# rueberger/MJHMC

Measured on AMD Instinct MI355X. Metric: particle-steps/sec (ndims x nparticles x L), higher is better.
Workload: dtype f64 state (ProductOfT: around the f32 matrix-core force)

## Files before the change

mjhmc_amd/csrc/api.hip:

```cpp
#include <hip/hip_runtime.h>

#include <algorithm>
#include <atomic>
#include <chrono>
#include <cmath>
#include <cstdio>
#include <cstdlib>
#include <cstring>
#include <string>
#include <thread>
#include <type_traits>
#include <vector>

#include "autocor.hpp"
#include "lagcov.hpp"
#include "handles.hpp"

static thread_local std::string g_err;

int mjhmc_fail(int code, const std::string& msg) {
  g_err = msg;
  return code;
}
static int fail(int code, const std::string& msg) { return mjhmc_fail(code, msg); }
// ... 180 lines not shown
    const int d = d0 + threadIdx.x;
    if (d < D && p < N) dst[(size_t)p * pitch + d] = (T)tile[threadIdx.x][pp];
  }
}

template <typename T>
__global__ void to_dim_major(const T* __restrict__ src, const int64_t* __restrict__ idx, double* __restrict__ dst,
                             int D, int64_t ncols, int pitch, int64_t rs, int64_t cs, int64_t off) {
  __shared__ double tile[32][33];
  const int64_t k0 = (int64_t)blockIdx.x * 32;
  const int d0 = blockIdx.y * 32;
#pragma unroll
  for (int i = 0; i < 4; ++i) {
    const int kk = threadIdx.y + 8 * i;
    const int64_t k = k0 + kk;
    const int d = d0 + threadIdx.x;
    if (d < D && k < ncols) {
      const int64_t row = idx ? idx[k] : k;
      tile[kk][threadIdx.x] = (double)src[(size_t)row * pitch + d];
    }
  }
  __syncthreads();
#pragma unroll
  for (int i = 0; i < 4; ++i) {
    const int dd = threadIdx.y + 8 * i;
    const int d = d0 + dd;
    const int64_t k = k0 + threadIdx.x;
    if (d < D && k < ncols) dst[(size_t)d * rs + (size_t)k * cs + off] = tile[threadIdx.x][dd];
  }
}

template <typename T>
__global__ void widen_vec(const T* __restrict__ src, double* __restrict__ dst, int64_t n) {
  const int64_t i = (int64_t)blockIdx.x * blockDim.x + threadIdx.x;
  if (i < n) dst[i] = (double)src[i];
}

template <typename T>
__global__ void flags_from_hflf(const T* __restrict__ h, uint8_t* __restrict__ out, int64_t n) {
  const int64_t i = (int64_t)blockIdx.x * blockDim.x + threadIdx.x;
  if (i < n) out[i] = (h[i] == h[i]) ? 1 : 0;
}

template <typename T>
__global__ void moments_kernel(const T* __restrict__ src, int64_t nrows_pad_per_slot, int64_t nrows_per_slot, int nslots,
                               int D, int pitch, double shift, double* out) {
  double s1 = 0.0, s2 = 0.0;
  const int64_t per_slot = nrows_per_slot * D;
  const int64_t total = per_slot * nslots;
  for (int64_t i = (int64_t)blockIdx.x * blockDim.x + threadIdx.x; i < total; i += (int64_t)gridDim.x * blockDim.x) {
    const int64_t slot = i / per_slot, rem = i - slot * per_slot;
    const int64_t row = rem / D;
    const int d = (int)(rem - row * D);
    const double v = (double)src[(size_t)(slot * nrows_pad_per_slot + row) * pitch + d] - shift;
    s1 += v;
    s2 += v * v;
  }
  for (int o = 32; o > 0; o >>= 1) {
    s1 += __shfl_xor(s1, o);
    s2 += __shfl_xor(s2, o);
  }
  __shared__ double sm[2][16];
  const int w = threadIdx.x >> 6;
  if ((threadIdx.x & 63) == 0) {
    sm[0][w] = s1;
    sm[1][w] = s2;
  }
  __syncthreads();
  if (threadIdx.x < 2) {
    double t = 0.0;
    for (int k = 0; k < (int)(blockDim.x >> 6); ++k) t += sm[threadIdx.x][k];
    atomicAdd(&out[threadIdx.x], t);
  }
}

template <typename T>
__global__ void narrow_vec(const double* __restrict__ src, T* __restrict__ dst, int64_t n) {
  const int64_t i = (int64_t)blockIdx.x * blockDim.x + threadIdx.x;
  if (i < n) dst[i] = (T)src[i];
}

constexpr int kColdChunk = 4096;
template <typename T>
struct ColdCache {
  const T* h;
  T* copy;
  __device__ bool operator()(int64_t p) const {
    const T v = h[p];
    copy[p] = v;
    return v != v;
  }
};
template <class Pred>
__global__ __launch_bounds__(1024) void compact_list_kernel(const Pred pred, int64_t N, const Control* ctl,
                                                            int* __restrict__ list, int* __restrict__ count) {
  __shared__ int hits[kColdChunk];
  __shared__ int n_hits, base;
  if (ctl->failed) return;
  if (threadIdx.x == 0) n_hits = 0;
  __syncthreads();
  const int lane = threadIdx.x & 63;
  for (int k = 0; k < kColdChunk / 1024; ++k) {
    const int64_t p = (int64_t)blockIdx.x * kColdChunk + k * 1024 + threadIdx.x;
    const bool cold = p < N && pred(p);
    const unsigned long long mask = __ballot(cold);
    if (mask) {
      int at = 0;
      if (lane == 0) at = atomicAdd(&n_hits, __popcll(mask));
      at = __shfl(at, 0);
      if (cold) hits[at + __popcll(mask & ((1ull << lane) - 1ull))] = (int)p;
    }
  }
  __syncthreads();
  if (threadIdx.x == 0) base = atomicAdd(count, n_hits);
  __syncthreads();
  for (int i = threadIdx.x; i < n_hits; i += 1024) list[base + i] = hits[i];
}

#define MJHMC_ENERGY_LAUNCHERS(NAME)                                               \
  struct NAME##_launchers {                                                        \
    template <class... A> static void jump(const A&... a) { NAME##_jump(a...); }  \
    template <class... A> static void leap(const A&... a) { NAME##_leap(a...); }  \
    template <class... A> static void step(const A&... a) { NAME##_step(a...); }  \
    template <class... A> static void eval(const A&... a) { NAME##_eval(a...); }  \
  };
MJHMC_ENERGY_LAUNCHERS(iso)
MJHMC_ENERGY_LAUNCHERS(diag)
MJHMC_ENERGY_LAUNCHERS(rough)
MJHMC_ENERGY_LAUNCHERS(mm)
MJHMC_ENERGY_LAUNCHERS(funnel_neal)
MJHMC_ENERGY_LAUNCHERS(funnel_ref)
#undef MJHMC_ENERGY_LAUNCHERS

template <class F>
static int with_elementwise_energy(int kind, F&& launch) {
  switch (kind) {
    case MJHMC_E_ISO_GAUSS: launch(iso_launchers{}); return 0;
    case MJHMC_E_DIAG_GAUSS: launch(diag_launchers{}); return 0;
    case MJHMC_E_ROUGH_WELL: launch(rough_launchers{}); return 0;
    case MJHMC_E_MM_GAUSS: launch(mm_launchers{}); return 0;
    case MJHMC_E_FUNNEL_NEAL: launch(funnel_neal_launchers{}); return 0;
    case MJHMC_E_FUNNEL_REF: launch(funnel_ref_launchers{}); return 0;
    default: return fail(MJHMC_ERR_UNSUPPORTED, "energy kind has no elementwise kernels");
  }
}

int ensure_stage(mjhmc_sampler* s, size_t elems) {
  if (s->stage_elems >= elems) return 0;
  if (s->stage) HIPCHK(hipFree(s->stage));
  s->stage = nullptr;
  s->stage_elems = 0;
  HIPCHK(hipMalloc(&s->stage, elems * sizeof(double)));
  s->stage_elems = elems;
  return 0;
}

static int upload_matrix(mjhmc_sampler* s, const double* host, void* dst) {
  TRY(ensure_stage(s, (size_t)s->D * s->N));
  HIPCHK(hipMemcpyAsync(s->stage, host, (size_t)s->D * s->N * sizeof(double), hipMemcpyHostToDevice, s->stream));
  dim3 grid((unsigned)((s->N + 31) / 32), (unsigned)((s->D + 31) / 32)), block(32, 8);
  if (s->dtype == MJHMC_F64)
    hipLaunchKernelGGL(to_particle_major<double>, grid, block, 0, s->stream, s->stage, (double*)dst, s->D, s->N,
                       s->sh.pitch);
  else if (s->dtype == MJHMC_BF16)
    hipLaunchKernelGGL(to_particle_major<__bf16>, grid, block, 0, s->stream, s->stage, (__bf16*)dst, s->D, s->N,
                       s->sh.pitch);
  else
    hipLaunchKernelGGL(to_particle_major<float>, grid, block, 0, s->stream, s->stage, (float*)dst, s->D, s->N,
                       s->sh.pitch);
  HIPCHK(hipGetLastError());
  return 0;
}

constexpr size_t kPipeChunk = (size_t)32 << 20;
constexpr int kCopyThreads = 8;

static int ensure_pipe(mjhmc_sampler* s) {
  for (int i = 0; i < 2; ++i) {
    if (!s->pipe_pin[i]) HIPCHK(hipHostMalloc(&s->pipe_pin[i], kPipeChunk, hipHostMallocDefault));
    if (!s->pipe_ev[i]) HIPCHK(hipEventCreateWithFlags(&s->pipe_ev[i], hipEventDisableTiming));
  }
  return 0;
}

int copy_to_host(mjhmc_sampler* s, const void* dev_src, void* host_dst, size_t bytes) {
  if (bytes < 2 * kPipeChunk) {
    HIPCHK(hipMemcpyAsync(host_dst, dev_src, bytes, hipMemcpyDeviceToHost, s->stream));
    HIPCHK(hipStreamSynchronize(s->stream));
    return 0;
  }
  TRY(ensure_pipe(s));
  const size_t nchunk = (bytes + kPipeChunk - 1) / kPipeChunk;
  auto issue = [&](size_t k) -> int {
    const size_t off = k * kPipeChunk, len = std::min(kPipeChunk, bytes - off);
    HIPCHK(hipMemcpyAsync(s->pipe_pin[k & 1], (const char*)dev_src + off, len, hipMemcpyDeviceToHost, s->stream));
    HIPCHK(hipEventRecord(s->pipe_ev[k & 1], s->stream));
    return 0;
  };
  TRY(issue(0));
  for (size_t k = 0; k < nchunk; ++k) {
    if (k + 1 < nchunk) TRY(issue(k + 1));
    HIPCHK(hipEventSynchronize(s->pipe_ev[k & 1]));
    const size_t off = k * kPipeChunk, len = std::min(kPipeChunk, bytes - off);
    const char* src = (const char*)s->pipe_pin[k & 1];
    char* dst = (char*)host_dst + off;
    const size_t slice = (len / kCopyThreads + 4095) / 4096 * 4096;
    std::thread th[kCopyThreads];
    int nth = 0;
    for (size_t o = slice; o < len; o += slice) {
      const size_t l = std::min(slice, len - o);
      th[nth++] = std::thread([=] { std::memcpy(dst + o, src + o, l); });
    }
    std::memcpy(dst, src, std::min(slice, len));
    for (int t = 0; t < nth; ++t) th[t].join();
  }
  return 0;
}

int download_cols(mjhmc_sampler* s, const void* src, const int64_t* dev_idx, int64_t ncols, double* host,
                  size_t host_elems, int64_t rs, int64_t cs, int64_t off, bool copy_out) {
  dim3 grid((unsigned)((ncols + 31) / 32), (unsigned)((s->D + 31) / 32)), block(32, 8);
  if (s->dtype == MJHMC_F64)
    hipLaunchKernelGGL(to_dim_major<double>, grid, block, 0, s->stream, (const double*)src, dev_idx, s->stage, s->D,
                       ncols, s->sh.pitch, rs, cs, off);
  else if (s->dtype == MJHMC_BF16 && !s->download_f32)
    hipLaunchKernelGGL(to_dim_major<__bf16>, grid, block, 0, s->stream, (const __bf16*)src, dev_idx, s->stage, s->D,
                       ncols, s->sh.pitch, rs, cs, off);
  else
    hipLaunchKernelGGL(to_dim_major<float>, grid, block, 0, s->stream, (const float*)src, dev_idx, s->stage, s->D,
                       ncols, s->sh.pitch, rs, cs, off);
  HIPCHK(hipGetLastError());
  if (copy_out) TRY(copy_to_host(s, s->stage, host, host_elems * sizeof(double)));
  return 0;
}

struct DlSession {
  std::vector<std::vector<hipEvent_t>> ev;
  std::atomic<int> marked{0};
  std::atomic<bool> launched{false};
  int n_iter = 0, ring_slot0 = 0;
  double* host = nullptr;
  int64_t n_total = 0, k0 = 0;
  std::atomic<int> downloaded{0};
  std::vector<char> retiled;
  std::atomic<bool> cancel{false};
  std::atomic<bool> exited{false};
  bool off = false;
  int rc = 0;
  std::string err;
};

static int dl_retile(mjhmc_sampler* s, const void* rows0, int64_t start, int64_t ncols, double* stage, hipStream_t st) {
  const char* src = (const char*)rows0 + (size_t)start * row_bytes(s);
  dim3 grid((unsigned)((ncols + 31) / 32), (unsigned)((s->D + 31) / 32)), block(32, 8);
  if (s->dtype == MJHMC_F64)
    hipLaunchKernelGGL(to_dim_major<double>, grid, block, 0, st, (const double*)src, (const int64_t*)nullptr, stage, s->D, ncols,
                       s->sh.pitch, s->N, (int64_t)1, start);
  else if (s->dtype == MJHMC_BF16)
    hipLaunchKernelGGL(to_dim_major<__bf16>, grid, block, 0, st, (const __bf16*)src, (const int64_t*)nullptr, stage, s->D, ncols,
                       s->sh.pitch, s->N, (int64_t)1, start);
  else
    hipLaunchKernelGGL(to_dim_major<float>, grid, block, 0, st, (const float*)src, (const int64_t*)nullptr, stage, s->D, ncols,
                       s->sh.pitch, s->N, (int64_t)1, start);
  HIPCHK(hipGetLastError());
  return 0;
}

static int dl_mark(mjhmc_sampler* s, int i0, int n, const hipStream_t* streams, int n_streams) {
  DlSession* d = s->dl;
  if (!d || d->off || i0 < d->marked.load(std::memory_order_acquire)) return 0;
  for (int i = i0; i < i0 + n && i < d->n_iter; ++i) {
    for (int k = 0; k < n_streams; ++k) {
      hipEvent_t e = nullptr;
      if (i == i0) {
        HIPCHK(hipEventCreateWithFlags(&e, hipEventDisableTiming));
        HIPCHK(hipEventRecord(e, streams[k]));
      } else {
        e = d->ev[(size_t)i0][(size_t)k];
      }
      d->ev[(size_t)i].push_back(e);
    }
  }
  d->marked.store(std::min(i0 + n, d->n_iter), std::memory_order_release);
  return 0;
}

static int dl_download_slot(mjhmc_sampler* s, DlSession* d, int i) {
  const size_t elems = (size_t)s->D * s->N;
  const size_t bytes = elems * sizeof(double), row = (size_t)s->N * sizeof(double);
  const void* src = (const char*)s->ring + (size_t)(d->ring_slot0 + i) * mat_bytes(s);
  const bool retiled = d->retiled[(size_t)i] != 0;
  const double* stage = retiled ? s->dl_stage + (size_t)i * elems : s->dl_stage;
  if (!retiled) TRY(dl_retile(s, src, 0, s->N, s->dl_stage, s->dl_stream));
  char* host = (char*)d->host;
  const size_t dst_row = (size_t)d->n_total * row, dst_off = (size_t)(d->k0 + i) * row;
  const size_t nchunk = (bytes + kPipeChunk - 1) / kPipeChunk;
  auto issue = [&](size_t k) -> int {
    const size_t off = k * kPipeChunk, len = std::min(kPipeChunk, bytes - off);
    HIPCHK(hipMemcpyAsync(s->dl_pin[k & 1], (const char*)stage + off, len, hipMemcpyDeviceToHost, s->dl_stream));
    HIPCHK(hipEventRecord(s->dl_ev[k & 1], s->dl_stream));
    return 0;
  };
  TRY(issue(0));
  for (size_t k = 0; k < nchunk; ++k) {
    if (k + 1 < nchunk) TRY(issue(k + 1));
    HIPCHK(hipEventSynchronize(s->dl_ev[k & 1]));
// ... 307 lines not shown
        for (int h = 0; h < 2; ++h)
          for (int i = 0; i < I; ++i)
            for (int j = 0; j < 8; ++j) {
              const int ws = ks / (2 * NB), b = (ks >> 1) % NB, sx = ks & 1;
              const int c = 32 * NB * ws + 32 * b + 16 * sx + 8 * (j >> 2) + 4 * h + (j & 3);
              a1[(((size_t)ks * 2 + h) * I + i) * 8 + j] = bf16_of(B[(size_t)i * C + c]);
            }
      for (int ks = 0; ks < 16; ++ks)
        for (int h = 0; h < 2; ++h)
          for (int c = 0; c < C; ++c)
            for (int j = 0; j < 8; ++j) {
              const int ws = ks >> 1, sx = ks & 1;
              const int i = 32 * ws + 16 * sx + 8 * (j >> 2) + 4 * h + (j & 3);
              a2[(((size_t)ks * 2 + h) * C + c) * 8 + j] = bf16_of(B[(size_t)i * C + c]);
            }
      std::vector<float> yv((size_t)P * I);
      for (size_t i = 0; i < yv.size(); ++i) yv[i] = (float)Y[i];
      const void* src[3] = {a1.data(), a2.data(), yv.data()};
      const size_t bytes[3] = {a1.size() * 2, a2.size() * 2, yv.size() * 4};
      e->sic_copies = kSicCopies;
      if (const char* cp = test_env("MJHMC_SIC_COPIES")) e->sic_copies = std::max(1, std::min(4, std::atoi(cp)));
      for (int i = 0; i < 3 && !rc; ++i) {
        const int reps = i < 2 ? e->sic_copies : 1;
        if (hipMalloc(&e->sic[i], bytes[i] * reps) != hipSuccess) rc = fail(MJHMC_ERR_HIP, "allocating SPARSE_CODE parameters failed");
        for (int r = 0; r < reps && !rc; ++r)
          if (hipMemcpy((char*)e->sic[i] + (size_t)r * bytes[i], src[i], bytes[i], hipMemcpyHostToDevice) != hipSuccess)
            rc = fail(MJHMC_ERR_HIP, "uploading SPARSE_CODE parameters failed");
      }
      break;
    }
    case MJHMC_E_HOST:
      if (nparams) rc = fail(MJHMC_ERR_INVALID, "HOST takes no parameters");
      break;
    default:
      rc = fail(MJHMC_ERR_UNSUPPORTED, "energy kind not implemented in this build");
  }
  if (rc) {
    mjhmc_energy_destroy(e);
    return rc;
  }
  *out = e;
  return 0;
}

int mjhmc_energy_create_expr_coupled(mjhmc_ctx* ctx, int ndims, const char* stat_exprs, const char* energy_expr,
                                     const char* energy0_expr, const char* grad_expr, const double* params, size_t nparams,
                                     const char* include_dir, mjhmc_energy** out) {
  if (!ctx || !out || !energy_expr || !grad_expr || !include_dir) return fail(MJHMC_ERR_INVALID, "NULL argument");
  if (ndims < 1) return fail(MJHMC_ERR_INVALID, "ndims must be >= 1");
  if (nparams && !params) return fail(MJHMC_ERR_INVALID, "params is NULL");
  HIPCHK(hipSetDevice(ctx->device));
  Shape sh;
  TRY(pick_shape(ndims, MJHMC_F64, &sh));
  mjhmc_energy* e = new mjhmc_energy();
  e->ctx = ctx;
  if (nparams) e->params.assign(params, params + nparams);
  std::memset(&e->ep, 0, sizeof(e->ep));
  e->ep.kind = MJHMC_E_USER_EXPR;
  e->ep.ndims = ndims;
  const int rc = user_energy_build(e, energy_expr, grad_expr, stat_exprs, energy0_expr, include_dir, params, nparams, sh.E);
  if (rc) {
    std::string keep = g_err;
    mjhmc_energy_destroy(e);
    g_err = keep;
    return rc;
  }
  *out = e;
  return 0;
}

int mjhmc_energy_create_expr(mjhmc_ctx* ctx, int ndims, const char* energy_expr, const char* grad_expr,
                             const double* params, size_t nparams, const char* include_dir, mjhmc_energy** out) {
  return mjhmc_energy_create_expr_coupled(ctx, ndims, nullptr, energy_expr, nullptr, grad_expr, params, nparams, include_dir, out);
}

int mjhmc_expr_check_coupled(int ndims, const char* stat_exprs, const char* energy_expr, const char* energy0_expr,
                             const char* grad_expr, const char* include_dir) {
  if (!energy_expr || !grad_expr || !include_dir) return fail(MJHMC_ERR_INVALID, "NULL argument");
  if (ndims < 1) return fail(MJHMC_ERR_INVALID, "ndims must be >= 1");
  Shape sh;
  TRY(pick_shape(ndims, MJHMC_F64, &sh));
  std::vector<char> code;
  std::vector<std::string> lowered;
  std::string err;
  const int rc = user_expr_compile(user_expr_source(energy_expr, grad_expr, stat_exprs ? stat_exprs : "", energy0_expr ? energy0_expr : ""),
                                   include_dir, sh.E, &code, &lowered, &err);
  return rc ? fail(rc, err) : 0;
}

int mjhmc_expr_check(int ndims, const char* energy_expr, const char* grad_expr, const char* include_dir) {
  return mjhmc_expr_check_coupled(ndims, nullptr, energy_expr, nullptr, grad_expr, include_dir);
}

int mjhmc_energy_create_linear(mjhmc_ctx* ctx, int ndims, int nexperts, const double* W, const double* b,
                               const char* energy_expr, const char* grad_expr, const double* params, size_t nparams,
                               const double* expert_params, int n_expert_rows, const char* include_dir, mjhmc_energy** out) {
  if (!ctx || !out) return fail(MJHMC_ERR_INVALID, "NULL argument");
  TRY(linear_check_args(ndims, nexperts, energy_expr, grad_expr, include_dir));
  if (!W || !b) return fail(MJHMC_ERR_INVALID, "W or b is NULL");
  if (nparams && !params) return fail(MJHMC_ERR_INVALID, "params is NULL");
  if (n_expert_rows < 0 || n_expert_rows > 4 || (n_expert_rows && !expert_params))
    return fail(MJHMC_ERR_INVALID, "LINEAR_EXPR takes 0 to 4 per-expert parameter rows");
  HIPCHK(hipSetDevice(ctx->device));
  mjhmc_energy* e = new mjhmc_energy();
  e->ctx = ctx;
  std::memset(&e->ep, 0, sizeof(e->ep));
  e->ep.kind = MJHMC_E_LINEAR_EXPR;
  e->ep.ndims = ndims;
  const int rc = linear_energy_build(e, nexperts, W, b, energy_expr, grad_expr, params, nparams, expert_params, n_expert_rows,
                                     include_dir);
  if (rc) {
    std::string keep = g_err;
    mjhmc_energy_destroy(e);
    g_err = keep;
    return rc;
  }
  *out = e;
  return 0;
}

int mjhmc_linear_check(int ndims, int nexperts, const char* energy_expr, const char* grad_expr, const char* include_dir) {
  TRY(linear_check_args(ndims, nexperts, energy_expr, grad_expr, include_dir));
  std::string err;
  const std::vector<char>* code = nullptr;
  const std::vector<std::string>* lowered = nullptr;
  const int rc = linear_compile(energy_expr, grad_expr, linear_dim(ndims, nexperts), include_dir, &err, &code, &lowered);
  return rc ? fail(rc, err) : 0;
}

int mjhmc_energy_destroy(mjhmc_energy* e) {
  if (!e) return 0;
  user_energy_free(e);
  linear_energy_free(e);
  if (e->dev64) (void)hipFree(e->dev64);
  if (e->dev32) (void)hipFree(e->dev32);
  for (float* q : e->pot)
    if (q) (void)hipFree(q);
  for (void* q : e->sic)
    if (q) (void)hipFree(q);
  delete e;
  return 0;
}

int mjhmc_sampler_destroy(mjhmc_sampler* s) {
  if (!s) return 0;
  (void)hipSetDevice(s->ctx->device);
  if (s->stream) (void)hipStreamSynchronize(s->stream);
  functionals_free_all(s);
  estimator_free_all(s);
  chainstats_free_all(s);
  histogram_free_all(s);
  pairhist_free_all(s);
  timegrid_free_all(s);
  void* ptrs[] = {s->flf_list, s->call_block, s->Hpre, s->Hwork, s->cold_list, s->pot64_scratch, s->Hspec[0], s->Hspec[1], s->Hspec_dump, s->Gbuf[0], s->Gbuf[1], s->Xbuf[0], s->Xbuf[1], s->Vbuf[0],  s->Vbuf[1], s->EX[0],     s->EX[1],  s->EV[0],
                  s->EV[1],   s->Hflf[0], s->Hflf[1],  s->dwell,  s->dwell_scratch,  s->trans,
                  s->ring,     s->dwell_ring, s->stage,  s->noise,  s->rexp,
                  s->runif,   s->scratch,  s->ck[0],    s->ck[1],    s->ck[2],   s->ck[3],  s->ck[4],
                  s->ck[5],   s->ck[6]};
  for (void* p : ptrs)
    if (p) (void)hipFree(p);
  for (auto& e : s->ev_total)
    if (e) (void)hipEventDestroy(e);
  for (auto& e : s->ev_k) (void)hipEventDestroy(e);
  for (auto& e : s->part_events) (void)hipEventDestroy(e);
  for (auto& q : s->part_streams) (void)hipStreamDestroy(q);
  if (s->ev_join) (void)hipEventDestroy(s->ev_join);
  if (s->ev_fork) (void)hipEventDestroy(s->ev_fork);
  for (void* q : s->ick)
    if (q) (void)hipFree(q);
  if (s->h_pin) (void)hipHostFree(s->h_pin);
  if (s->dl_stage) (void)hipFree(s->dl_stage);
  for (int i = 0; i < 2; ++i) {
    if (s->dl_pin[i]) (void)hipHostFree(s->dl_pin[i]);
    if (s->dl_ev[i]) (void)hipEventDestroy(s->dl_ev[i]);
  }
  if (s->dl_stream) (void)hipStreamDestroy(s->dl_stream);
  for (int i = 0; i < 2; ++i) {
    if (s->pipe_pin[i]) (void)hipHostFree(s->pipe_pin[i]);
    if (s->pipe_ev[i]) (void)hipEventDestroy(s->pipe_ev[i]);
  }
  host_traj_free(s);
  if (s->stream) (void)hipStreamDestroy(s->stream);
  delete s;
  return 0;
}

int mjhmc_sampler_create(mjhmc_ctx* ctx, mjhmc_energy* e, int64_t nparticles, int64_t first_particle_id, int dtype,
                         const double* Xinit, const double* Vinit, uint64_t seed, int mode, mjhmc_sampler** out) {
  if (!ctx || !e || !out || !Xinit) return fail(MJHMC_ERR_INVALID, "NULL argument");
  if (nparticles < 1) return fail(MJHMC_ERR_INVALID, "nparticles must be >= 1");
  if (dtype != MJHMC_F64 && dtype != MJHMC_F32 && dtype != MJHMC_BF16)
    return fail(MJHMC_ERR_INVALID, "dtype must be F64, F32 or BF16");
  if (dtype == MJHMC_BF16 && !e->is_sic()) return fail(MJHMC_ERR_UNSUPPORTED, "BF16 state: SPARSE_CODE only");
  if (e->is_sic() && dtype == MJHMC_F64)
    return fail(MJHMC_ERR_UNSUPPORTED, "SPARSE_CODE runs with BF16 state (the benchmark's) or F32 state (the reference's)");
  if (e->is_user() && dtype != MJHMC_F64) return fail(MJHMC_ERR_UNSUPPORTED, "user-expression energies run in float64");
  if (e->is_host() && dtype != MJHMC_F64) return fail(MJHMC_ERR_UNSUPPORTED, "host-evaluated energies run in float64");
  if (mode < MJHMC_MODE_MJHMC || mode > MJHMC_MODE_CTHMC) return fail(MJHMC_ERR_INVALID, "unknown sampler mode");
  if (first_particle_id < 0 || first_particle_id + nparticles > 0xFFFFFFFFLL)
    return fail(MJHMC_ERR_INVALID, "global particle ids must fit 32 bits");
  HIPCHK(hipSetDevice(ctx->device));
  mjhmc_sampler* s = new mjhmc_sampler();
  s->ctx = ctx;
  s->en = e;
  s->N = nparticles;
  s->Npad = (nparticles + 63) / 64 * 64;
  s->first_pid = first_particle_id;
  s->D = e->ep.ndims;
  s->dtype = dtype;
  s->mode = mode;
  s->seed = seed;
  int rc = shape_for(e, &s->dtype, &s->sh);
  if (rc) {
    delete s;
    return rc;
  }
  dtype = s->dtype;
  auto build = [&]() -> int {
    HIPCHK(hipStreamCreateWithFlags(&s->stream, hipStreamNonBlocking));
    const size_t mb = mat_bytes(s);
    for (int i = 0; i < 2; ++i) {
      HIPCHK(hipMalloc(&s->Xbuf[i], mb));
      HIPCHK(hipMalloc(&s->Vbuf[i], mb));
      HIPCHK(hipMemsetAsync(s->Xbuf[i], 0, mb, s->stream));
      HIPCHK(hipMemsetAsync(s->Vbuf[i], 0, mb, s->stream));
      if (e->is_pot() || ((e->is_host() || s->sh.wide) && i == 0)) {
        HIPCHK(hipMalloc(&s->Gbuf[i], mb));
        HIPCHK(hipMemsetAsync(s->Gbuf[i], 0, mb, s->stream));
      }
      if (e->is_dense()) {
        if (!s->Hwork) {
          HIPCHK(hipMalloc((void**)&s->Hwork, s->Npad * ssize(s)));
          HIPCHK(hipMemsetAsync(s->Hwork, 0, s->Npad * ssize(s), s->stream));
          HIPCHK(hipMalloc((void**)&s->cold_list, (2 * s->Npad + 3 * kMaxDenseParts) * sizeof(int)));
          if (e->is_pot() && dtype == MJHMC_F64 && !e->pot_big())
            HIPCHK(hipMalloc((void**)&s->pot64_scratch, (size_t)kMaxDenseParts * pot64_scratch_workgroups() * 2 * 32 * row_bytes(s)));
        }
        HIPCHK(hipMalloc(&s->Hspec[i], s->Npad * ssize(s)));
        HIPCHK(hipMemsetAsync(s->Hspec[i], 0xFF, s->Npad * ssize(s), s->stream));
      }
      HIPCHK(hipMalloc(&s->EX[i], s->Npad * ssize(s)));
      HIPCHK(hipMalloc(&s->EV[i], s->Npad * ssize(s)));
      HIPCHK(hipMalloc(&s->Hflf[i], s->Npad * ssize(s)));
      HIPCHK(hipMemsetAsync(s->EX[i], 0, s->Npad * ssize(s), s->stream));
      HIPCHK(hipMemsetAsync(s->EV[i], 0, s->Npad * ssize(s), s->stream));
      HIPCHK(hipMemsetAsync(s->Hflf[i], 0xFF, s->Npad * ssize(s), s->stream));
    }
    HIPCHK(hipMalloc((void**)&s->dwell, s->Npad * sizeof(double)));
    HIPCHK(hipMemsetAsync(s->dwell, 0, s->Npad * sizeof(double), s->stream));
    HIPCHK(hipMalloc((void**)&s->dwell_scratch, s->Npad * sizeof(double)));
    HIPCHK(hipMalloc((void**)&s->trans, s->Npad));
    HIPCHK(hipMemsetAsync(s->trans, 0, s->Npad, s->stream));
    TRY(ensure_call_block(s, 1024));
    HIPCHK(hipEventCreate(&s->ev_total[0]));
    HIPCHK(hipEventCreate(&s->ev_total[1]));
    if ((size_t)s->D * s->N * sizeof(double) >= 2 * kPipeChunk) TRY(ensure_pipe(s));
    s->Xcur = s->Xbuf[0];
    TRY(upload_matrix(s, Xinit, s->Xcur));
    if (s->sh.round32) TRY(round_rows32(s, s->Xcur));
    if (Vinit) {
      TRY(upload_matrix(s, Vinit, s->Vbuf[0]));
      if (s->sh.round32) TRY(round_rows32(s, s->Vbuf[0]));
      TRY(run_eval(s, s->Xcur, s->Gbuf[0], s->EX[0], s->Vbuf[0], nullptr, s->EV[0]));
    } else {
      TRY(run_eval(s, s->Xcur, s->Gbuf[0], s->EX[0], nullptr, s->Vbuf[0], s->EV[0]));
      if (s->sh.round32) {
        TRY(round_rows32(s, s->Vbuf[0]));
        TRY(run_eval(s, nullptr, nullptr, nullptr, s->Vbuf[0], nullptr, s->EV[0]));
      }
    }
    HIPCHK(hipStreamSynchronize(s->stream));
    return 0;
  };
  rc = build();
  if (rc) {
    std::string keep = g_err;
    mjhmc_sampler_destroy(s);
    g_err = keep;
    return rc;
  }
  *out = s;
  return 0;
}

static int drop_spec(mjhmc_sampler* s) {
  if (!s->Hspec[0]) return 0;
  HIPCHK(hipSetDevice(s->ctx->device));
  HIPCHK(hipMemsetAsync(s->Hspec[s->scur], 0xFF, (size_t)s->Npad * ssize(s), s->stream));
  return 0;
}

int mjhmc_set_hparams(mjhmc_sampler* s, double epsilon, int num_leapfrog_steps, double p_r, double beta,
                      double p_flip) {
  if (!s) return fail(MJHMC_ERR_INVALID, "sampler is NULL");
  if (num_leapfrog_steps < 0) return fail(MJHMC_ERR_INVALID, "num_leapfrog_steps must be >= 0");
  if (epsilon != s->eps || num_leapfrog_steps != s->L) TRY(drop_spec(s));
  s->eps = epsilon;
  s->L = num_leapfrog_steps;
  s->p_r = p_r;
  s->beta = beta;
  s->p_flip = p_flip;
  return 0;
}

int mjhmc_checkpoint(mjhmc_sampler* s) {
  if (!s) return fail(MJHMC_ERR_INVALID, "sampler is NULL");
  HIPCHK(hipSetDevice(s->ctx->device));
  const size_t mb = mat_bytes(s), vb = (size_t)s->Npad * ssize(s), db = (size_t)s->Npad * sizeof(double);
  const int nck = (s->en->is_pot() || s->en->is_host() || s->sh.wide) ? 7 : 6;
  const size_t sizes[7] = {mb, mb, vb, vb, vb, db, mb};
  const void* src[7] = {s->Xcur, s->Vbuf[s->vcur], s->EX[s->scur], s->EV[s->scur], s->Hflf[s->scur], s->dwell,
                        s->Gbuf[s->vcur]};
  for (int i = 0; i < nck; ++i) {
    if (!s->ck[i]) HIPCHK(hipMalloc(&s->ck[i], sizes[i]));
    HIPCHK(hipMemcpyAsync(s->ck[i], src[i], sizes[i], hipMemcpyDeviceToDevice, s->stream));
  }
  s->ck_tick = s->tick;
  s->ck_valid = true;
  return 0;
}

int mjhmc_restore(mjhmc_sampler* s) {
  if (!s) return fail(MJHMC_ERR_INVALID, "sampler is NULL");
  if (!s->ck_valid) return fail(MJHMC_ERR_INVALID, "no checkpoint taken");
  HIPCHK(hipSetDevice(s->ctx->device));
  const size_t mb = mat_bytes(s), vb = (size_t)s->Npad * ssize(s), db = (size_t)s->Npad * sizeof(double);
  const int nck = (s->en->is_pot() || s->en->is_host() || s->sh.wide) ? 7 : 6;
  const size_t sizes[7] = {mb, mb, vb, vb, vb, db, mb};
  s->Xcur = s->Xbuf[0];
  void* dst[7] = {s->Xcur, s->Vbuf[s->vcur], s->EX[s->scur], s->EV[s->scur], s->Hflf[s->scur], s->dwell,
                  s->Gbuf[s->vcur]};
  for (int i = 0; i < nck; ++i) HIPCHK(hipMemcpyAsync(dst[i], s->ck[i], sizes[i], hipMemcpyDeviceToDevice, s->stream));
  TRY(drop_spec(s));
  s->list_valid = false;
  s->tick = s->ck_tick;
  s->undo_valid = false;
  HIPCHK(hipStreamSynchronize(s->stream));
  return 0;
}

int mjhmc_rollback(mjhmc_sampler* s) {
  if (!s) return fail(MJHMC_ERR_INVALID, "sampler is NULL");
  if (!s->undo_valid) return fail(MJHMC_ERR_INVALID, "nothing to roll back: the last call was not a committed single iteration");
  s->undo_valid = false;
  s->list_valid = false;
  if (s->undo_multipass) return multipass_rollback(s);
  s->Xcur = s->undo_X;
  s->vcur ^= 1;
  s->scur ^= 1;
  return 0;
}

int mjhmc_get_tick(mjhmc_sampler* s, uint64_t* tick) {
  if (!s || !tick) return fail(MJHMC_ERR_INVALID, "NULL argument");
  *tick = s->tick;
  return 0;
}

int mjhmc_set_tick(mjhmc_sampler* s, uint64_t tick) {
  if (!s) return fail(MJHMC_ERR_INVALID, "sampler is NULL");
  s->tick = tick;
  s->undo_valid = false;
  return 0;
}

int mjhmc_advance_tick(mjhmc_sampler* s, int64_t n) {
  if (!s || n < 0) return fail(MJHMC_ERR_INVALID, "bad argument");
  s->tick += (uint64_t)n;
  return 0;
}

int mjhmc_reset_flf_cache(mjhmc_sampler* s) {
  if (!s) return fail(MJHMC_ERR_INVALID, "sampler is NULL");
  HIPCHK(hipSetDevice(s->ctx->device));
  HIPCHK(hipMemsetAsync(s->Hflf[s->scur], 0xFF, s->Npad * ssize(s), s->stream));
  s->list_valid = false;
  return drop_spec(s);
}

}

static void fill_iter_stats(const mjhmc_sampler* s, const std::vector<long long>& hs, int attempts, int done, bool failed,
                            mjhmc_iter_stats* per_iter) {
  if (!per_iter) return;
  for (int i = 0; i < attempts; ++i) {
    mjhmc_iter_stats& st = per_iter[i];
    std::memset(&st, 0, sizeof(st));
    if (s->mode == MJHMC_MODE_MJHMC) {
      st.l = hs[4 * i + 0];
      st.f = hs[4 * i + 1];
      st.r = hs[4 * i + 2];
      st.n_cold = hs[4 * i + 3] & 0xFFFFFFFFLL;
    } else if (s->mode == MJHMC_MODE_CTHMC) {
      st.fl = hs[4 * i + 0];
      st.f = hs[4 * i + 1];
      st.r = hs[4 * i + 2];
    } else {
      st.l = hs[4 * i + 0];
      st.f = hs[4 * i + 1];
      st.r = hs[4 * i + 2];
      st.fl = hs[4 * i + 3];
    }
    st.E_evals = s->N + st.n_cold;
    st.dEdX_evals = (int64_t)s->L * (s->N + st.n_cold);
    st.nonfinite = (failed && i == done) ? 1 : 0;
    st.L_used = s->L;
    st.eps_used = s->eps;
    st.n_flf_run = (s->mode == MJHMC_MODE_MJHMC && s->en->is_dense()) ? (hs[4 * i + 3] >> 32) : st.n_cold;
  }
}

template <class A>
struct IsDenseJump : std::false_type {};
template <typename S, typename H, bool POT>
struct IsDenseJump<DenseJumpArgs<S, H, POT>> : std::true_type {};

template <class A>
static A part_args(const A& a, int64_t start, int64_t n, int64_t npad, size_t pitch, int which, int* counters) {
  A h = a;
  h.X_in = a.X_in + (size_t)start * pitch;
  h.V_in = a.V_in + (size_t)start * pitch;
  h.X_out = a.X_out + (size_t)start * pitch;
  h.V_out = a.V_out + (size_t)start * pitch;
  h.EX_in = a.EX_in + start;
  h.EV_in = a.EV_in + start;
  h.Hflf_in = a.Hflf_in + start;
  h.EX_out = a.EX_out + start;
  h.EV_out = a.EV_out + start;
  h.Hflf_out = a.Hflf_out + start;
  h.dwell = a.dwell + start;
  h.dwell_ring = a.dwell_ring + start;
  h.trans = a.trans + start;
  if constexpr (IsDenseJump<A>::value) {
    h.Hspec_in = a.Hspec_in + start;
    h.Hwork = a.Hwork + start;
    h.Hspec_out = a.Hspec_out + start;
    h.cold_list = a.cold_list + start;
    h.next_list = a.next_list + start;
    h.cold_count = counters + 3 * which + a.iter % 3;
    h.next_count = counters + 3 * which + (a.iter + 1) % 3;
    h.zero_count = counters + 3 * which + (a.iter + 2) % 3;
    if constexpr (A::kPot) {
      h.G_in = a.G_in + (size_t)start * pitch;
      h.G_out = a.G_out + (size_t)start * pitch;
    }
    if constexpr (A::kScratch)
      h.scratch = a.scratch + (size_t)which * pot64_scratch_workgroups() * 2 * 32 * (size_t)pitch;
  }
  h.N = n;
  h.Npad = npad;
  h.first_pid = a.first_pid + start;
  return h;
}

static int ensure_part_streams(mjhmc_sampler* s, int n_parts) {
  if (!s->ev_fork) {
    HIPCHK(hipEventCreateWithFlags(&s->ev_fork, hipEventDisableTiming));
    HIPCHK(hipEventCreateWithFlags(&s->ev_join, hipEventDisableTiming));
  }
  while ((int)s->part_streams.size() < n_parts - 1) {
    hipStream_t q;
    hipEvent_t e;
    HIPCHK(hipStreamCreateWithFlags(&q, hipStreamNonBlocking));
    s->part_streams.push_back(q);
    HIPCHK(hipEventCreateWithFlags(&e, hipEventDisableTiming));
    s->part_events.push_back(e);
  }
  return 0;
}

static int split_state_copy(mjhmc_sampler* s, bool restore) {
  const size_t mb = mat_bytes(s), vb = (size_t)s->Npad * ssize(s), db = (size_t)s->Npad * sizeof(double);
  const int nck = s->en->is_pot() ? 7 : 6;
  const size_t sizes[7] = {mb, mb, vb, vb, vb, db, mb};
  void* live[7] = {s->Xcur, s->Vbuf[s->vcur], s->EX[s->scur], s->EV[s->scur], s->Hflf[s->scur], s->dwell, s->Gbuf[s->vcur]};
  for (int i = 0; i < nck; ++i) {
    if (!s->ick[i]) HIPCHK(hipMalloc(&s->ick[i], sizes[i]));
    if (restore) HIPCHK(hipMemcpyAsync(live[i], s->ick[i], sizes[i], hipMemcpyDeviceToDevice, s->stream));
    else HIPCHK(hipMemcpyAsync(s->ick[i], live[i], sizes[i], hipMemcpyDeviceToDevice, s->stream));
  }
  if (restore) TRY(drop_spec(s));
  return 0;
}

static int read_back_call(mjhmc_sampler* s, size_t stats_rows, Control* hc, long long* hs, int* counts = nullptr, int n_counts = 0) {
  const size_t head = kCtlBytes + counts_bytes(s->stats_cap);
  const size_t need = head + stats_rows * 4 * sizeof(long long);
  if (s->h_pin_cap < need) {
    if (s->h_pin) HIPCHK(hipHostFree(s->h_pin));
    s->h_pin = nullptr;
    s->h_pin_cap = 0;
    HIPCHK(hipHostMalloc((void**)&s->h_pin, need * 2, hipHostMallocDefault));
    s->h_pin_cap = need * 2;
  }
  HIPCHK(hipMemcpyAsync(s->h_pin, s->call_block, need, hipMemcpyDeviceToHost, s->stream));
  HIPCHK(hipStreamSynchronize(s->stream));
  std::memcpy(hc, s->h_pin, sizeof(Control));
  if (counts) std::memcpy(counts, s->h_pin + kCtlBytes, (size_t)n_counts * sizeof(int));
  std::memcpy(hs, s->h_pin + head, stats_rows * 4 * sizeof(long long));
  return 0;
}

template <class A>
static A jump_args(const mjhmc_sampler* s, int iter, int vi, int si, const void* xin, void* xout, int ring_slot0,
                   long long* stats) {
  using S = std::remove_pointer_t<decltype(A::X_out)>;
  using H = std::remove_pointer_t<decltype(A::EX_out)>;
  A a{};
  a.X_in = (const S*)xin;
  a.V_in = (const S*)s->Vbuf[vi];
  a.X_out = (S*)xout;
  a.V_out = (S*)s->Vbuf[vi ^ 1];
  a.EX_in = (const H*)s->EX[si];
  a.EV_in = (const H*)s->EV[si];
  a.Hflf_in = (const H*)s->Hflf[si];
  a.EX_out = (H*)s->EX[si ^ 1];
  a.EV_out = (H*)s->EV[si ^ 1];
  a.Hflf_out = (H*)s->Hflf[si ^ 1];
  a.dwell = s->dwell;
  a.dwell_ring = ring_slot0 >= 0 ? s->dwell_ring + (size_t)(ring_slot0 + iter) * s->Npad : s->dwell_scratch;
  a.trans = s->trans;
  a.ctl = s->ctl;
  a.stats = (unsigned long long*)stats;
  a.N = s->N;
  a.Npad = s->Npad;
  a.first_pid = s->first_pid;
  a.L = s->L;
  a.iter = iter;
  a.mode = s->mode;
  a.eps = (H)s->eps;
  a.chalf = (H)(-s->eps / 2.);
  a.r_keep = (H)std::sqrt(1. - s->beta);
  a.r_mix = (H)std::sqrt(s->beta);
  a.p_r = s->p_r;
  a.p_flip = s->p_flip;
  a.key = rng_key(s, s->tick + (uint64_t)iter);
  if constexpr (!IsDenseJump<A>::value) {
    a.D = s->D;
    a.pitch = s->sh.pitch;
    a.CH = s->sh.CH;
    a.logG = s->sh.logG;
    a.ab = ab_flags() | (fused_rows(s) ? 0 : kAbNoRows);
  } else if constexpr (A::kPot) {
    a.D = s->D;
  }
  return a;
}

static int move_out_of_ring(mjhmc_sampler* s, int slot0, int n) {
  const size_t mb = mat_bytes(s);
  const char* lo = (const char*)s->ring + (size_t)slot0 * mb;
  if ((const char*)s->Xcur >= lo && (const char*)s->Xcur < lo + (size_t)n * mb) {
    HIPCHK(hipMemcpyAsync(s->Xbuf[0], s->Xcur, mb, hipMemcpyDeviceToDevice, s->stream));
    s->Xcur = s->Xbuf[0];
  }
  return 0;
}

template <typename T, class StreamOf>
static int debug_poison(mjhmc_sampler* s, int iter, int si, StreamOf stream_of) {
  const char* poison = test_env("MJHMC_DEBUG_POISON");
  int pit = -1;
  long long pp = -1;
  if (!poison || std::sscanf(poison, "%d:%lld", &pit, &pp) != 2 || pit != iter || pp < 0 || pp >= s->N) return 0;
  static const double nan64 = __builtin_nan("");
  static const float nan32 = __builtin_nanf("");
  const hipStream_t pst = stream_of(pp);
  if (pst != s->stream && iter == 0) HIPCHK(hipStreamSynchronize(s->stream));
  HIPCHK(hipMemcpyAsync((char*)s->EV[si] + (size_t)pp * ssize(s), sizeof(T) == 8 ? (const void*)&nan64 : (const void*)&nan32,
                        ssize(s), hipMemcpyHostToDevice, pst));
  return 0;
}

template <typename T>
static int iterate_fused_t(mjhmc_sampler* s, int n_iter, int ring_slot0, mjhmc_iter_stats* per_iter, int* n_done) {
  const size_t mb = mat_bytes(s);
  const int need = n_iter + kMaxFuse;
  TRY(zero_call(s, need));

  if (ring_slot0 >= 0) TRY(move_out_of_ring(s, ring_slot0, n_iter));
  void* xin = s->Xcur;
  struct Launch {
    int i0, K, vi, si;
    void* xin;
    void* xout;
  };
  int64_t split_at = 0;
  int n_parts = 3;
  bool allow_split_now = true;
  if (ring_slot0 < 0 && !test_env("MJHMC_NO_SPLIT")) {
    if (const char* np = test_env("MJHMC_SPLIT_PARTS")) n_parts = std::max(2, std::min(8, std::atoi(np)));
    const int64_t nslots = s->Npad >> (6 - s->sh.logG);
    if (nslots >= 8 * 4096 && !fused_rows(s)) split_at = (s->Npad / n_parts) / 256 * 256;
    if (split_at <= 0 || split_at * (n_parts - 1) >= s->N) split_at = 0;
    if (split_at) TRY(ensure_part_streams(s, n_parts));
  }
  auto launch = [&](const Launch& l, long long* stats) -> int {
    JumpArgs<T> a = jump_args<JumpArgs<T>>(s, l.i0, l.vi, l.si, l.xin, l.xout, ring_slot0, stats);
    a.n_fuse = l.K;
    if (ring_slot0 >= 0) {
      a.xiter = (T*)((char*)s->ring + (size_t)(ring_slot0 + l.i0) * mb);
      a.xiter_stride = mb / sizeof(T);
    }
    if (split_at > 0 && allow_split_now) {
      HIPCHK(hipEventRecord(s->ev_fork, s->stream));
      for (int k = 0; k < n_parts; ++k) {
        const int64_t start = (int64_t)k * split_at, stop = (k + 1 == n_parts) ? a.N : start + split_at;
        const JumpArgs<T> h = part_args(a, start, stop - start, (k + 1 == n_parts) ? a.Npad - start : split_at, (size_t)a.pitch, k, nullptr);
        hipStream_t q = k == 0 ? s->stream : s->part_streams[(size_t)k - 1];
        if (k > 0) HIPCHK(hipStreamWaitEvent(q, s->ev_fork, 0));
        TRY(with_elementwise_energy(s->en->ep.kind, [&](auto en) { en.jump(h, s->en->ep, s->sh.E, q); }));
        if (k > 0) {
          HIPCHK(hipEventRecord(s->part_events[(size_t)k - 1], q));
          HIPCHK(hipStreamWaitEvent(s->stream, s->part_events[(size_t)k - 1], 0));
        }
      }
    } else {
      TRY(with_elementwise_energy(s->en->ep.kind, [&](auto en) { en.jump(a, s->en->ep, s->sh.E, s->stream); }));
    }
    HIPCHK(hipGetLastError());
    return 0;
  };
  auto out_of = [&](int i0, int K, void* in) -> void* {
    if (ring_slot0 >= 0) return (char*)s->ring + (size_t)(ring_slot0 + i0 + K - 1) * mb;
    return (in != s->Xbuf[0]) ? s->Xbuf[0] : s->Xbuf[1];
  };

// ... 335 lines not shown
  a.logG = w.sh.logG;
  a.L = L;
  a.eps = (T)eps;
  a.chalf = (T)(-eps / 2.);
  if constexpr (sizeof(T) == 8) {
    if (w.en->is_user()) return user_launch_leap(w.en, a, w.stream);
  }
  TRY(with_elementwise_energy(w.en->ep.kind, [&](auto en) { en.leap(a, w.en->ep, w.sh.E, w.stream); }));
  HIPCHK(hipGetLastError());
  return 0;
}

template <typename S, bool POT>
static int leap_dense(mjhmc_sampler& w, void* const* buf, double eps, int L) {
  DenseLeapArgs<S, POT> a{};
  a.X = (const S*)buf[0];
  a.V = (const S*)buf[1];
  a.X_out = (S*)buf[2];
  a.V_out = (S*)buf[3];
  a.G = (float*)buf[4];
  a.EX = (float*)buf[5];
  a.EV = (float*)buf[6];
  a.N = w.N;
  a.ntiles = dense_ntiles(&w, w.N, w.Npad);
  a.L = L;
  a.eps = (float)eps;
  a.chalf = (float)(-eps / 2.);
  if constexpr (POT) {
    a.D = w.D;
    pot_launch_leap(a, w.en->pot_model(), w.stream, w.en->pot_gen());
  } else {
    sic_launch_leap(a, w.en->sic_model(), w.stream);
  }
  HIPCHK(hipGetLastError());
  return 0;
}

extern "C" {

int mjhmc_iterate(mjhmc_sampler* s, int n_iter, const double* replay_normal, const double* replay_exp,
                  const double* replay_unif, int ring_slot0, mjhmc_iter_stats* per_iter, int* n_done) {
  if (!s) return fail(MJHMC_ERR_INVALID, "sampler is NULL");
  if (n_iter < 1) return fail(MJHMC_ERR_INVALID, "n_iter must be >= 1");
  if (s->mode == MJHMC_MODE_CONTROL) {
    if ((replay_normal == nullptr) != (replay_unif == nullptr) || replay_exp)
      return fail(MJHMC_ERR_INVALID, "CONTROL replay takes replay_normal and replay_unif together");
  } else if ((replay_normal == nullptr) != (replay_exp == nullptr) || replay_unif) {
    return fail(MJHMC_ERR_INVALID, "jump-process replay takes replay_normal and replay_exp together");
  }
  if (ring_slot0 >= 0 && (!s->ring || ring_slot0 + n_iter > s->ring_slots))
    return fail(MJHMC_ERR_INVALID, "ring slots out of range (call mjhmc_ring_alloc)");
  if (s->en->is_host())
    return fail(MJHMC_ERR_UNSUPPORTED, "a host-evaluated energy is driven step by step: mjhmc_traj_begin / _step / _finish");
  HIPCHK(hipSetDevice(s->ctx->device));
  const bool pot64_fused = s->sh.wide && s->en->is_pot() && !s->en->pot_big() && !s->sh.round32 && s->L >= 1 &&
                           !test_env("MJHMC_POT64_MULTIPASS");
  if (s->sh.wide && !pot64_fused) {
    s->list_valid = false;
    const int rc = multipass_iterate(s, n_iter, replay_normal, replay_exp, replay_unif, ring_slot0, per_iter, n_done);
    if (rc == 0) TRY(drop_spec(s));
    return rc;
  }
  return s->dtype == MJHMC_F64
             ? iterate_t<double>(s, n_iter, replay_normal, replay_exp, replay_unif, ring_slot0, per_iter, n_done)
             : iterate_t<float>(s, n_iter, replay_normal, replay_exp, replay_unif, ring_slot0, per_iter, n_done);
}

int mjhmc_iterate_download(mjhmc_sampler* s, int n_iter, int ring_slot0, double* host_out, int64_t n_total, int64_t k0,
                           mjhmc_iter_stats* per_iter, int* n_done) {
  if (!s || !host_out || n_iter < 1) return fail(MJHMC_ERR_INVALID, "bad argument");
  if (ring_slot0 < 0 || !s->ring || ring_slot0 + n_iter > s->ring_slots)
    return fail(MJHMC_ERR_INVALID, "ring slots out of range (call mjhmc_ring_alloc)");
  if (k0 < 0 || k0 + n_iter > n_total) return fail(MJHMC_ERR_INVALID, "time indices [k0, k0 + n_iter) outside the host array");
  HIPCHK(hipSetDevice(s->ctx->device));
  if (!s->dl_stream) {
    int lo = 0, hi = 0;
    HIPCHK(hipDeviceGetStreamPriorityRange(&lo, &hi));
    HIPCHK(hipStreamCreateWithPriority(&s->dl_stream, hipStreamNonBlocking, hi));
  }
  const size_t elems = (size_t)s->D * s->N;
  if (s->dl_stage_elems < (size_t)n_iter * elems) {
    double* big = nullptr;
    if (hipMalloc((void**)&big, (size_t)n_iter * elems * sizeof(double)) == hipSuccess) {
      if (s->dl_stage) HIPCHK(hipFree(s->dl_stage));
      s->dl_stage = big;
      s->dl_stage_elems = (size_t)n_iter * elems;
    } else {
      (void)hipGetLastError();
      if (s->dl_stage_elems < elems) {
        if (s->dl_stage) HIPCHK(hipFree(s->dl_stage));
        s->dl_stage = nullptr;
        s->dl_stage_elems = 0;
        HIPCHK(hipMalloc((void**)&s->dl_stage, elems * sizeof(double)));
        s->dl_stage_elems = elems;
      }
    }
  }
  for (int i = 0; i < 2; ++i) {
    if (!s->dl_pin[i]) HIPCHK(hipHostMalloc(&s->dl_pin[i], kPipeChunk, hipHostMallocDefault));
    if (!s->dl_ev[i]) HIPCHK(hipEventCreateWithFlags(&s->dl_ev[i], hipEventDisableTiming));
  }
  DlSession d;
  d.ev.resize((size_t)n_iter);
  d.retiled.assign((size_t)n_iter, 0);
  d.n_iter = n_iter;
  d.ring_slot0 = ring_slot0;
  d.host = host_out;
  d.n_total = n_total;
  d.k0 = k0;
  s->dl = &d;
  std::thread worker(dl_worker, s, &d);
  int done = 0;
  const int rc = mjhmc_iterate(s, n_iter, nullptr, nullptr, nullptr, ring_slot0, per_iter, &done);
  d.launched.store(true, std::memory_order_release);
  worker.join();
  s->dl = nullptr;
  int rc2 = d.rc;
  if (rc2) g_err = d.err;
  if (!rc && !rc2) {
    HIPCHK(hipStreamSynchronize(s->dl_stream));
    for (int i = d.downloaded.load(); i < done && !rc2; ++i) rc2 = dl_download_slot(s, &d, i);
  }
  dl_destroy_events(&d);
  if (n_done) *n_done = done;
  return rc ? rc : rc2;
}

static int read_vec(mjhmc_sampler* s, const void* dev, void* host, size_t nbytes) {
  if (nbytes != (size_t)s->N * sizeof(double)) return fail(MJHMC_ERR_INVALID, "expected N float64");
  if (s->dtype == MJHMC_F64) {
    HIPCHK(hipMemcpyAsync(host, dev, nbytes, hipMemcpyDeviceToHost, s->stream));
  } else {
    TRY(ensure_stage(s, (size_t)s->N));
    hipLaunchKernelGGL(widen_vec<float>, dim3((unsigned)((s->N + 255) / 256)), dim3(256), 0, s->stream,
                       (const float*)dev, s->stage, s->N);
    HIPCHK(hipGetLastError());
    HIPCHK(hipMemcpyAsync(host, s->stage, nbytes, hipMemcpyDeviceToHost, s->stream));
  }
  HIPCHK(hipStreamSynchronize(s->stream));
  return 0;
}

int mjhmc_read(mjhmc_sampler* s, int field, void* host_dst, size_t nbytes) {
  if (!s || !host_dst) return fail(MJHMC_ERR_INVALID, "NULL argument");
  HIPCHK(hipSetDevice(s->ctx->device));
  const size_t mat = (size_t)s->D * s->N;
  switch (field) {
    case MJHMC_F_X:
    case MJHMC_F_V:
    case MJHMC_F_DEDX: {
      if (nbytes != mat * sizeof(double)) return fail(MJHMC_ERR_INVALID, "expected (D,N) float64");
      TRY(ensure_stage(s, mat));
      const void* src = field == MJHMC_F_X ? s->Xcur : s->Vbuf[s->vcur];
      if (field == MJHMC_F_DEDX && (s->en->is_pot() || s->en->is_host() || s->sh.wide)) {
        src = s->Gbuf[s->vcur];
      } else if (field == MJHMC_F_DEDX && s->en->is_sic()) {
        if (!s->scratch) HIPCHK(hipMalloc(&s->scratch, (size_t)s->Npad * s->D * sizeof(float)));
        TRY(run_eval(s, s->Xcur, s->scratch, nullptr, nullptr, nullptr, nullptr));
        s->download_f32 = true;
        const int rc = download_cols(s, s->scratch, nullptr, s->N, (double*)host_dst, mat, s->N, 1, 0, true);
        s->download_f32 = false;
        return rc;
      } else if (field == MJHMC_F_DEDX) {
        if (!s->scratch) HIPCHK(hipMalloc(&s->scratch, mat_bytes(s)));
        TRY(run_eval(s, s->Xcur, s->scratch, nullptr, nullptr, nullptr, nullptr));
        src = s->scratch;
      }
      return download_cols(s, src, nullptr, s->N, (double*)host_dst, mat, s->N, 1, 0, true);
    }
    case MJHMC_F_EX: return read_vec(s, s->EX[s->scur], host_dst, nbytes);
    case MJHMC_F_EV: return read_vec(s, s->EV[s->scur], host_dst, nbytes);
    case MJHMC_F_HFLF: return read_vec(s, s->Hflf[s->scur], host_dst, nbytes);
    case MJHMC_F_DWELL:
      if (nbytes != (size_t)s->N * sizeof(double)) return fail(MJHMC_ERR_INVALID, "expected N float64");
      HIPCHK(hipMemcpyAsync(host_dst, s->dwell, nbytes, hipMemcpyDeviceToHost, s->stream));
      HIPCHK(hipStreamSynchronize(s->stream));
      return 0;
    case MJHMC_F_CACHE: {
      if (nbytes != (size_t)s->N) return fail(MJHMC_ERR_INVALID, "expected N uint8");
      TRY(ensure_stage(s, (size_t)(s->N + 7) / 8));
      uint8_t* flags = (uint8_t*)s->stage;
      const dim3 g((unsigned)((s->N + 255) / 256)), b(256);
      if (s->dtype == MJHMC_F64)
        hipLaunchKernelGGL(flags_from_hflf<double>, g, b, 0, s->stream, (const double*)s->Hflf[s->scur], flags, s->N);
      else
        hipLaunchKernelGGL(flags_from_hflf<float>, g, b, 0, s->stream, (const float*)s->Hflf[s->scur], flags, s->N);
      HIPCHK(hipGetLastError());
      HIPCHK(hipMemcpyAsync(host_dst, flags, nbytes, hipMemcpyDeviceToHost, s->stream));
      HIPCHK(hipStreamSynchronize(s->stream));
      return 0;
    }
    case MJHMC_F_TRANS:
      if (nbytes != (size_t)s->N) return fail(MJHMC_ERR_INVALID, "expected N uint8");
      HIPCHK(hipMemcpyAsync(host_dst, s->trans, nbytes, hipMemcpyDeviceToHost, s->stream));
      HIPCHK(hipStreamSynchronize(s->stream));
      return 0;
    default: return fail(MJHMC_ERR_INVALID, "unknown field");
  }
}

int mjhmc_write(mjhmc_sampler* s, int field, const void* host_src, size_t nbytes) {
  if (!s || !host_src) return fail(MJHMC_ERR_INVALID, "NULL argument");
  HIPCHK(hipSetDevice(s->ctx->device));
  const size_t mat = (size_t)s->D * s->N;
  switch (field) {
    case MJHMC_F_X:
    case MJHMC_F_V: {
      if (nbytes != mat * sizeof(double)) return fail(MJHMC_ERR_INVALID, "expected (D,N) float64");
      void* dst = field == MJHMC_F_X ? s->Xcur : s->Vbuf[s->vcur];
      s->undo_valid = false;
      s->list_valid = false;
      if (field == MJHMC_F_X) s->host_energy_set = false;
      TRY(upload_matrix(s, (const double*)host_src, dst));
      if (s->sh.round32) TRY(round_rows32(s, dst));
      TRY(run_eval(s, s->Xcur, s->Gbuf[s->vcur], s->EX[s->scur], s->Vbuf[s->vcur], nullptr, s->EV[s->scur]));
      HIPCHK(hipMemsetAsync(s->Hflf[s->scur], 0xFF, s->Npad * ssize(s), s->stream));
      TRY(drop_spec(s));
      HIPCHK(hipStreamSynchronize(s->stream));
      return 0;
    }
    case MJHMC_F_HFLF: {
      if (nbytes != (size_t)s->N * sizeof(double)) return fail(MJHMC_ERR_INVALID, "expected N float64");
      TRY(drop_spec(s));
      s->list_valid = false;
      if (s->dtype == MJHMC_F64) {
        HIPCHK(hipMemcpyAsync(s->Hflf[s->scur], host_src, nbytes, hipMemcpyHostToDevice, s->stream));
      } else {
        TRY(ensure_stage(s, (size_t)s->N));
        HIPCHK(hipMemcpyAsync(s->stage, host_src, nbytes, hipMemcpyHostToDevice, s->stream));
        hipLaunchKernelGGL(narrow_vec<float>, dim3((unsigned)((s->N + 255) / 256)), dim3(256), 0, s->stream,
                           (const double*)s->stage, (float*)s->Hflf[s->scur], s->N);
        HIPCHK(hipGetLastError());
      }
      HIPCHK(hipStreamSynchronize(s->stream));
      return 0;
    }
    default: return fail(MJHMC_ERR_INVALID, "field is not writable");
  }
}

int mjhmc_ring_alloc(mjhmc_sampler* s, int n_slots) {
  if (!s || n_slots < 1) return fail(MJHMC_ERR_INVALID, "bad argument");
  HIPCHK(hipSetDevice(s->ctx->device));
  if (n_slots <= s->ring_slots) return 0;
  HIPCHK(hipStreamSynchronize(s->stream));
  const size_t mb = mat_bytes(s);
  void* ring = nullptr;
  double* dring = nullptr;
  hipError_t e = hipMalloc(&ring, (size_t)n_slots * mb);
  if (e == hipSuccess) e = hipMalloc((void**)&dring, (size_t)n_slots * s->Npad * sizeof(double));
  if (e != hipSuccess) {
    if (ring) (void)hipFree(ring);
    (void)hipGetLastError();
    size_t free_b = 0, total_b = 0;
    (void)hipMemGetInfo(&free_b, &total_b);
    char msg[320];
    std::snprintf(msg, sizeof(msg), "a sample ring of %d slots x %.3f GB = %.1f GB does not fit the device (%.1f GB free of %.1f GB): "
                  "record in chunks (mjhmc_iterate_download over a smaller ring) -- the ring the sampler had is kept",
                  n_slots, mb / 1e9, (double)n_slots * mb / 1e9, free_b / 1e9, total_b / 1e9);
    return fail(MJHMC_ERR_HIP, msg);
  }
  HIPCHK(hipMemsetAsync(ring, 0, (size_t)n_slots * mb, s->stream));
  HIPCHK(hipStreamSynchronize(s->stream));
  s->undo_valid = false;
  if (s->ring && (char*)s->Xcur >= (char*)s->ring && (char*)s->Xcur < (char*)s->ring + (size_t)s->ring_slots * mb) {
    HIPCHK(hipMemcpy(s->Xbuf[0], s->Xcur, mb, hipMemcpyDeviceToDevice));
    s->Xcur = s->Xbuf[0];
  }
  if (s->ring) HIPCHK(hipFree(s->ring));
  if (s->dwell_ring) HIPCHK(hipFree(s->dwell_ring));
  s->ring = ring;
  s->dwell_ring = dring;
  s->ring_slots = n_slots;
  ++s->ring_gen;
  return 0;
}

int mjhmc_ring_slot_bytes(mjhmc_sampler* s, uint64_t* bytes) {
  if (!s || !bytes) return fail(MJHMC_ERR_INVALID, "NULL argument");
  *bytes = (uint64_t)mat_bytes(s) + (uint64_t)s->Npad * sizeof(double);
  return 0;
}

int mjhmc_mem_info(mjhmc_ctx* ctx, uint64_t* free_bytes, uint64_t* total_bytes) {
  if (!ctx || !free_bytes || !total_bytes) return fail(MJHMC_ERR_INVALID, "NULL argument");
  HIPCHK(hipSetDevice(ctx->device));
  size_t f = 0, t = 0;
  HIPCHK(hipMemGetInfo(&f, &t));
  *free_bytes = f;
  *total_bytes = t;
  return 0;
}

int mjhmc_ring_read_dwell(mjhmc_sampler* s, int slot0, int n, double* host_dst) {
  if (!s || !host_dst) return fail(MJHMC_ERR_INVALID, "NULL argument");
  if (slot0 < 0 || n < 1 || slot0 + n > s->ring_slots) return fail(MJHMC_ERR_INVALID, "slots out of range");
  HIPCHK(hipSetDevice(s->ctx->device));
  HIPCHK(hipMemcpy2DAsync(host_dst, (size_t)s->N * sizeof(double), s->dwell_ring + (size_t)slot0 * s->Npad,
                          (size_t)s->Npad * sizeof(double), (size_t)s->N * sizeof(double), (size_t)n,
                          hipMemcpyDeviceToHost, s->stream));
  HIPCHK(hipStreamSynchronize(s->stream));
  return 0;
}

int mjhmc_ring_gather(mjhmc_sampler* s, const int64_t* idx, int64_t n, double* host_out) {
  if (!s || !idx || !host_out || n < 1) return fail(MJHMC_ERR_INVALID, "bad argument");
  HIPCHK(hipSetDevice(s->ctx->device));
  const int64_t pool = (int64_t)s->ring_slots * s->N;
  for (int64_t k = 0; k < n; ++k)
    if (idx[k] < 0 || idx[k] >= pool) return fail(MJHMC_ERR_INVALID, "gather index outside the sample ring");
  std::vector<int64_t> rows((size_t)n);
  for (int64_t k = 0; k < n; ++k) rows[k] = (idx[k] / s->N) * s->Npad + idx[k] % s->N;
  int64_t* didx = nullptr;
  HIPCHK(hipMalloc((void**)&didx, n * sizeof(int64_t)));
  int rc = 0;
  do {
    if (hipMemcpyAsync(didx, rows.data(), n * sizeof(int64_t), hipMemcpyHostToDevice, s->stream) != hipSuccess) {
      rc = fail(MJHMC_ERR_HIP, "index upload failed");
      break;
    }
    rc = ensure_stage(s, (size_t)s->D * n);
    if (rc) break;
    rc = download_cols(s, s->ring, didx, n, host_out, (size_t)s->D * n, n, 1, 0, true);
  } while (0);
  (void)hipFree(didx);
  return rc;
}

int mjhmc_ring_read(mjhmc_sampler* s, int slot0, int n, int stacked, double* host_out) {
  if (!s || !host_out) return fail(MJHMC_ERR_INVALID, "NULL argument");
  if (slot0 < 0 || n < 1 || slot0 + n > s->ring_slots) return fail(MJHMC_ERR_INVALID, "slots out of range");
  HIPCHK(hipSetDevice(s->ctx->device));
  const size_t total = (size_t)s->D * s->N * n;
  TRY(ensure_stage(s, total));
  const size_t mb = mat_bytes(s);
  const char* base = (const char*)s->ring + (size_t)slot0 * mb;
  if (!stacked) {
    for (int k = 0; k < n; ++k)
      TRY(download_cols(s, base + (size_t)k * mb, nullptr, s->N, host_out, total, (int64_t)n * s->N, 1,
                        (int64_t)k * s->N, k == n - 1));
  } else {
    for (int k = 0; k < n; ++k)
      TRY(download_cols(s, base + (size_t)k * mb, nullptr, s->N, host_out, total, (int64_t)s->N * n, n, k, k == n - 1));
  }
  return 0;
}

#ifdef MJHMC_TEST_HOOKS
extern "C" int mjhmc_test_ring_write(mjhmc_sampler* s, int slot, const double* X) {
  if (!s || !X || slot < 0 || slot >= s->ring_slots) return fail(MJHMC_ERR_INVALID, "bad argument");
  char* dst = (char*)s->ring + (size_t)slot * mat_bytes(s);
  if ((char*)s->Xcur == dst) return fail(MJHMC_ERR_INVALID, "the slot holds the live state");
  HIPCHK(hipSetDevice(s->ctx->device));
  if (s->undo_valid && (char*)s->undo_X == dst) s->undo_valid = false;
  TRY(upload_matrix(s, X, dst));
  HIPCHK(hipStreamSynchronize(s->stream));
  return 0;
}
#endif

int mjhmc_ring_moments(mjhmc_sampler* s, int slot0, int n, double shift, double* sum, double* sumsq) {
  if (!s || !sum || !sumsq) return fail(MJHMC_ERR_INVALID, "NULL argument");
  if (slot0 < 0 || n < 1 || slot0 + n > s->ring_slots) return fail(MJHMC_ERR_INVALID, "slots out of range");
  HIPCHK(hipSetDevice(s->ctx->device));
  TRY(ensure_stage(s, 2));
  HIPCHK(hipMemsetAsync(s->stage, 0, 2 * sizeof(double), s->stream));
  const char* base = (const char*)s->ring + (size_t)slot0 * mat_bytes(s);
  const dim3 grid(1024), block(256);
// ... 267 lines not shown
```

mjhmc_amd/csrc/dense_pot.hpp:

```cpp
#pragma once
#ifndef __HIPCC_RTC__
#include <hip/hip_runtime.h>
#endif
#include <stdint.h>

#include "elementwise.hpp"

namespace mjhmc {

constexpr int kPotDim = 512;

struct PotModel {
  const float* W1;
  const float* W2T;
  const float* cb;
  const float* alpha;
  int dim;
  int ndims;
};

using PotJumpArgs = DenseJumpArgs<float, float, true>;
using Pot64JumpArgs = DenseJumpArgs<double, double, true>;
using PotLeapArgs = DenseLeapArgs<float, true>;
using PotEvalArgs = DenseEvalArgs<float, true>;

struct PotLinear {
  const float* q;
  const float* p;
  int K;
  int stride;
};

template <bool REPLAY>
__device__ __forceinline__ int dense_decide(float H0, float HL, float Hflf, double p_r, uint32_t pid, int64_t p,
                                            int64_t N, const double* rexp, const RngKey& key, double& dwell, bool& bad) {
  const double l_rate = sqrt(exp((double)(H0 - HL)));
  const double flf_rate = sqrt(exp((double)(H0 - Hflf)));
  const double mn = (flf_rate != flf_rate || l_rate != l_rate) ? __builtin_nan("") : fmin(flf_rate, l_rate);
  const double f_rate = flf_rate - mn;
  const double r_rate = p_r;
  double eL, eF, eR;
  if constexpr (REPLAY) {
    eL = rexp[p];
    eF = rexp[N + p];
    eR = rexp[2 * N + p];
  } else {
    const u32x4 wq = philox4x32_10(pid, key.tick_lo, key.tick_hi, kSlotExpLF, key.k0, key.k1);
    const u32x4 qq = philox4x32_10(pid, key.tick_lo, key.tick_hi, kSlotExpR, key.k0, key.k1);
    eL = -log(u53(wq.w0, wq.w1));
    eF = -log(u53(wq.w2, wq.w3));
    eR = -log(u53(qq.w0, qq.w1));
  }
  bad = !(isfinite(l_rate) && isfinite(f_rate) && isfinite(r_rate));
  const double dL = l_rate == 0.0 ? __builtin_huge_val() : (1.0 / l_rate) * eL;
  const double dF = f_rate == 0.0 ? __builtin_huge_val() : (1.0 / f_rate) * eF;
  const double dR = r_rate == 0.0 ? __builtin_huge_val() : (1.0 / r_rate) * eR;
  int k = 0;
  double best = dL;
  if (!(best != best) && (dF < best || dF != dF)) {
    k = 1;
    best = dF;
  }
  if (!(best != best) && (dR < best || dR != dR)) {
    k = 2;
    best = dR;
  }
  dwell = best;
  return k;
}

template <bool REPLAY>
__device__ __forceinline__ int dense_decide_ct(float H0, float HL, double p_r, uint32_t pid, int64_t p, int64_t N,
                                               const double* rexp, const RngKey& key, double& dwell, bool& bad) {
  const double fl_rate = sqrt(exp((double)(H0 - HL)));
  const double r_rate = p_r;
  double eFL, eF, eR;
  if constexpr (REPLAY) {
    eFL = rexp[p];
    eF = rexp[N + p];
    eR = rexp[2 * N + p];
  } else {
    const u32x4 wq = philox4x32_10(pid, key.tick_lo, key.tick_hi, kSlotExpLF, key.k0, key.k1);
    const u32x4 qq = philox4x32_10(pid, key.tick_lo, key.tick_hi, kSlotExpR, key.k0, key.k1);
    eFL = -log(u53(wq.w0, wq.w1));
    eF = -log(u53(wq.w2, wq.w3));
    eR = -log(u53(qq.w0, qq.w1));
  }
  bad = !(isfinite(fl_rate) && isfinite(r_rate));
  const double dFL = fl_rate == 0.0 ? __builtin_huge_val() : (1.0 / fl_rate) * eFL;
  const double dF = eF;
  const double dR = r_rate == 0.0 ? __builtin_huge_val() : (1.0 / r_rate) * eR;
  int kk = 0;
  double best = dF;
  if (!(best != best) && (dFL < best || dFL != dFL)) {
    kk = 1;
    best = dFL;
  }
  if (!(best != best) && (dR < best || dR != dR)) {
    kk = 2;
    best = dR;
  }
  dwell = best;
  return kk == 0 ? 1 : (kk == 1 ? 0 : 2);
}

template <bool REPLAY>
__device__ __forceinline__ int dense_control(float H0, float HL, double p_r, double p_flip, uint32_t pid, int64_t p,
                                             int64_t N, const double* runif, const RngKey& key, bool& gate) {
  double uacc, uflip, ugate;
  if constexpr (REPLAY) {
    uacc = runif[p];
    uflip = runif[N + p];
    ugate = runif[2 * N];
  } else {
    const u32x4 q = philox4x32_10(pid, key.tick_lo, key.tick_hi, kSlotExpR, key.k0, key.k1);
    const u32x4 f = philox4x32_10(pid, key.tick_lo, key.tick_hi, kSlotFlip, key.k0, key.k1);
    const u32x4 g = philox4x32_10(0xFFFFFFFFu, key.tick_lo, key.tick_hi, kSlotFlip, key.k0, key.k1);
    uacc = u53(q.w2, q.w3);
    uflip = u53(f.w0, f.w1);
    ugate = u53(g.w2, g.w3);
  }
  const double dH = (double)(H0 - HL);
  const bool accept = !(dH < 0.0) || (uacc < exp(dH));
  const bool flip = uflip < p_flip;
  gate = ugate < p_r;
  return (accept ? 1 : 0) | (flip ? 2 : 0);
}

__device__ __forceinline__ void normal_pair_f32(const RngKey& k, uint32_t pid, uint32_t pair, float& z0, float& z1) {
  const u32x4 w = philox4x32_10(pid, k.tick_lo, k.tick_hi, pair, k.k0, k.k1);
  const float u1 = (float)u53(w.w0, w.w1);
  const float u2 = (float)u53(w.w2, w.w3);
  const float r = sqrtf(-2.0f * logf(u1 > 0.f ? u1 : 1e-38f));
  float s, c;
  sincospif(2.0f * u2, &s, &c);
  z0 = r * c;
  z1 = r * s;
}

struct PotBigModel {
  const float* W1b;
  const float* W2Tb;
  const float* cb;
  const float* alpha;
  int dim;
  int ndims;
};
#ifndef __HIPCC_RTC__
void pot_big_eval(const PotBigModel& m, const float* X32, float* G32, float* E32, float* U, int64_t rows_pad, hipStream_t st);

struct PotGenerated {
  hipFunction_t jump32[3][2] = {};
  hipFunction_t jump64[3][2] = {};
  hipFunction_t eval = nullptr, leap = nullptr;
  PotLinear lin{};
};

void pot_launch_jump(const PotJumpArgs& a, const PotModel& mdl, hipStream_t st, const PotGenerated* gen = nullptr);
void pot_launch_eval(const PotEvalArgs& a, const PotModel& mdl, hipStream_t st, const PotGenerated* gen = nullptr);
void pot_launch_leap(const PotLeapArgs& a, const PotModel& mdl, hipStream_t st, const PotGenerated* gen = nullptr);
void pot64_launch_jump(const Pot64JumpArgs& a, const PotModel& mdl, hipStream_t st, const PotGenerated* gen = nullptr);
template <class A>
inline void pot_launch_generated(hipFunction_t f, unsigned grid, hipStream_t st, const A& a, const PotModel& mdl, const PotLinear& lin) {
  void* params[] = {(void*)&a, (void*)&mdl, (void*)&lin};
  (void)hipModuleLaunchKernel(f, grid, 1, 1, 256, 1, 1, 0, st, params, nullptr);
}
int pot64_scratch_workgroups();
#endif

}
```

mjhmc_amd/csrc/dense_pot64.hip:

```cpp
#include <hip/hip_runtime.h>
#include <stdint.h>

#include <algorithm>

#include "dense_pot.hpp"
#include "dense_pot64_kernels.hpp"
#include "dense_pot_tile.hpp"

namespace mjhmc {

__global__ void pot64_cold_list_kernel(const double* __restrict__ Hflf_in, const double* __restrict__ Hspec_in, int64_t N,
                                       int* __restrict__ list, int* __restrict__ count, const Control* ctl) {
  if (ctl->failed) return;
  const int64_t p = (int64_t)blockIdx.x * blockDim.x + threadIdx.x;
  const double hc = p < N ? Hflf_in[p] : 0.0, hs = p < N ? Hspec_in[p] : 0.0;
  append_cold(list, count, (p < N) && !(hc == hc) && !(hs == hs), p);
}

template <int NB, bool REPLAY, int MODE>
__global__ __launch_bounds__(256, 1) void pot64_jump_kernel(const Pot64JumpArgs a, const PotModel mdl) {
  const PotExperts xp;
#include "dense_pot64_jump.inc"
}

template <int NB, bool REPLAY>
__global__ __launch_bounds__(256) void pot64_decide_kernel(const Pot64JumpArgs a) {
  __shared__ Finish64Shared<NB> sh;
  if (a.ctl->failed) return;
  const int w = threadIdx.x >> 6, c = threadIdx.x & 31, h = (threadIdx.x & 63) >> 5;
  unsigned n0 = 0, n1 = 0, n2 = 0, n3 = 0;
  bool any_bad = false;
  for (int64_t tile = blockIdx.x; tile < a.ntiles; tile += gridDim.x) {
    const int64_t p = tile * kP + c;
    const bool alive = p < a.N;
    if (w == 0 && h == 0) {
      const int64_t pp = alive ? p : 0;
      const uint32_t pid = (uint32_t)(a.first_pid + pp);
      const double EX0 = a.EX_in[p], EV0 = a.EV_in[p];
      const double H0 = EX0 + EV0;
      const double HL = a.EX_out[p] + a.EV_out[p];
      double Hflf = a.Hflf_in[p];
      const bool cold = !(Hflf == Hflf);
      if (cold) {
        Hflf = a.Hspec_in[p];
        if (!(Hflf == Hflf)) Hflf = a.Hwork[p];
      }
      double best = 0.0;
      bool bad = false, gate = false;
      const int k = pot64_decide<REPLAY, kModeMJHMC>(a, H0, HL, Hflf, pp, pid, best, bad, gate);
      sh.s.move[c] = alive ? k : 0;
      any_bad |= bad && alive;
      append_cold(a.next_list, a.next_count, alive && k == 2, p);
      a.dwell[p] = best;
      a.dwell_ring[p] = best;
      a.trans[p] = (uint8_t)k;
      if (alive) {
        n0 += (k == 0);
        n1 += (k == 1);
        n2 += (k == 2);
        n3 += cold;
      }
      if (k != 0) {
        a.EX_out[p] = EX0;
        a.EV_out[p] = EV0;
      }
      a.Hflf_out[p] = k == 0 ? H0 : __builtin_nan("");
      a.Hspec_out[p] = k == 1 ? HL : __builtin_nan("");
    }
    __syncthreads();
    if (__syncthreads_or(sh.s.move[c] != 0)) {
      const size_t roff = (size_t)p * (128 * NB) + 32 * NB * w + 4 * NB * h;
      VTile<NB> v;
      Tile<NB> g;
      pot64_finish<NB, REPLAY, kModeMJHMC, true>(a, sh, p, alive, roff, w, c, h, v, g);
      __syncthreads();
    }
  }
  if (any_bad) {
    a.ctl->failed = 1;
    a.ctl->failed_iter = a.iter;
  }
  __shared__ unsigned tally[4];
  if (threadIdx.x < 4) tally[threadIdx.x] = 0;
  __syncthreads();
  if (n0) atomicAdd(&tally[0], n0);
  if (n1) atomicAdd(&tally[1], n1);
  if (n2) atomicAdd(&tally[2], n2);
  if (n3) atomicAdd(&tally[3], n3);
  __syncthreads();
  if (threadIdx.x < 4 && tally[threadIdx.x]) atomicAdd(&a.stats[threadIdx.x], (unsigned long long)tally[threadIdx.x]);
}

static int resident_cus64() {
  int dev = 0, cus = 0;
  (void)hipGetDevice(&dev);
  (void)hipDeviceGetAttribute(&cus, hipDeviceAttributeMultiprocessorCount, dev);
  return std::max(1, cus);
}

int pot64_scratch_workgroups() { return resident_cus64(); }

template <int NB, int MODE>
static void launch64_mode(const Pot64JumpArgs& a, const PotModel& mdl, unsigned grid, hipStream_t st, const PotGenerated* gen) {
  const bool replay = MODE == kModeControl ? (a.runif && a.noise) : (a.rexp && a.noise);
  if (gen) pot_launch_generated(gen->jump64[MODE][replay ? 1 : 0], grid, st, a, mdl, gen->lin);
  else if (replay) hipLaunchKernelGGL((pot64_jump_kernel<NB, true, MODE>), dim3(grid), dim3(256), 0, st, a, mdl);
  else hipLaunchKernelGGL((pot64_jump_kernel<NB, false, MODE>), dim3(grid), dim3(256), 0, st, a, mdl);
}

template <int NB>
static void launch64_nb(const Pot64JumpArgs& a, const PotModel& mdl, hipStream_t st, const PotGenerated* gen) {
  const int cus = resident_cus64();
  if (a.mode == kModeMJHMC) {
    if (a.iter == 0 || a.rescan) {
      (void)hipMemsetAsync(std::min(a.cold_count, std::min(a.next_count, a.zero_count)), 0, 3 * sizeof(int), st);
      hipLaunchKernelGGL(pot64_cold_list_kernel, dim3((unsigned)((a.N + 255) / 256)), dim3(256), 0, st, a.Hflf_in, a.Hspec_in,
                         a.N, a.cold_list, a.cold_count, (const Control*)a.ctl);
    }
    const unsigned grid = (unsigned)std::min<int64_t>(2 * a.ntiles, cus);
    launch64_mode<NB, kModeMJHMC>(a, mdl, grid, st, gen);
    const unsigned fgrid = (unsigned)std::min<int64_t>(a.ntiles, 4 * cus);
    if (a.rexp && a.noise) hipLaunchKernelGGL((pot64_decide_kernel<NB, true>), dim3(fgrid), dim3(256), 0, st, a);
    else hipLaunchKernelGGL((pot64_decide_kernel<NB, false>), dim3(fgrid), dim3(256), 0, st, a);
  } else {
    const unsigned grid = (unsigned)std::min<int64_t>(a.ntiles, cus);
    if (a.mode == kModeCT) launch64_mode<NB, kModeCT>(a, mdl, grid, st, gen);
    else launch64_mode<NB, kModeControl>(a, mdl, grid, st, gen);
  }
}

void pot64_launch_jump(const Pot64JumpArgs& a, const PotModel& mdl, hipStream_t st, const PotGenerated* gen) {
  if (mdl.dim == 128) launch64_nb<1>(a, mdl, st, gen);
  else if (mdl.dim == 256) launch64_nb<2>(a, mdl, st, gen);
  else launch64_nb<4>(a, mdl, st, gen);
}

#ifdef POT_STAMPS
}
extern "C" int mjhmc_pot64_stamps(unsigned long long* out) {
  return (int)hipMemcpyFromSymbol(out, HIP_SYMBOL(mjhmc::g_pot_stamp), sizeof(mjhmc::g_pot_stamp));
}
extern "C" int mjhmc_pot64_item_stamps(unsigned long long* out) {
  return (int)hipMemcpyFromSymbol(out, HIP_SYMBOL(mjhmc::g_pot_istamp), sizeof(mjhmc::g_pot_istamp));
}
namespace mjhmc {
#endif

}
```

mjhmc_amd/csrc/dense_pot64_jump.inc:

```
  __shared__ Shared64<NB> sh;
  if (a.ctl->failed) return;
  const int lane = threadIdx.x & 63, w = threadIdx.x >> 6, c = lane & 31, h = lane >> 5;
  const int ncold = MODE == kModeMJHMC ? *a.cold_count : 0;
  const int64_t nft = (ncold + kP - 1) / kP;
  if ((int64_t)blockIdx.x >= nft + a.ntiles) return;
  if (MODE == kModeMJHMC && blockIdx.x == 0 && threadIdx.x == 0) {
    *a.zero_count = 0;
    if (ncold) atomicAdd(&a.stats[3], (unsigned long long)ncold << 32);
  }
  __shared__ unsigned tally[5];
  if (threadIdx.x < 5) tally[threadIdx.x] = 0;
  AReg<NB> ar;
  areg_load<NB>(mdl, w, c, h, ar);
  stage_bias<NB>(mdl, sh.s);
  const Work<NB> wk = work_of<NB>(a.scratch, blockIdx.x, w, lane);
  for (int64_t item = blockIdx.x; item < nft + a.ntiles; item += gridDim.x) {
    const bool inverse = item < nft;
    [[maybe_unused]] const int istamp_item = (int)(item / gridDim.x) & 15;
    auto column_of = [&](int64_t it) -> int64_t {
      if (it < nft) {
        const int64_t slot = it * kP + c;
        return a.cold_list[slot < ncold ? slot : ncold - 1];
      }
      return (it - nft) * kP + c;
    };
    Tile<NB> g;
    VTile<NB> v;
    float exl = 0.f;
    double EVL;
    {
      const int64_t p = column_of(item);
      POT_ISTAMP(0);
      staged_start<NB>(sh.s, wk, a.X_in, a.V_in, a.G_in, p, w, c, h, g, v, inverse);
      POT_ISTAMP(1);
      EVL = pot64_trajectory<NB>(mdl, xp, ar, sh, w, c, h, lane, wk, g, v, a.L, a.eps, a.chalf, &exl);
      POT_ISTAMP(2);
    }
    int64_t item_again = item;
    asm volatile("" : "+s"(item_again));
    const int64_t p = column_of(item_again);
    const bool alive = p < a.N;
    const size_t roff = (size_t)p * (128 * NB) + 32 * NB * w + 4 * NB * h;
    if (!inverse) staged_end_x<NB>(sh.s, wk, a.X_out, p, w, c, h);
    POT_ISTAMP(3);
    const double EXL = (double)exl;
    const double HL = EXL + EVL;
    if (inverse) {
      if (w == 0 && h == 0) a.Hwork[p] = HL;
      __syncthreads();
      POT_ISTAMP(4);
      continue;
    }

    if constexpr (MODE == kModeMJHMC) {
      if (w == 0 && h == 0) {
        a.EX_out[p] = EXL;
        a.EV_out[p] = EVL;
      }
      staged_end_vg<NB>(sh.s, a.V_out, a.G_out, p, w, c, h, v, g);
      POT_ISTAMP(4);
      continue;
    }

    if (w == 0 && h == 0) {
      const int64_t pp = alive ? p : 0;
      const uint32_t pid = (uint32_t)(a.first_pid + pp);
      const double EX0 = a.EX_in[p], EV0 = a.EV_in[p];
      const double H0 = EX0 + EV0;
      double best = 0.0;
      bool bad = false, gate = false;
      const int k = pot64_decide<REPLAY, MODE>(a, H0, HL, 0.0, pp, pid, best, bad, gate);
      if (bad && alive) tally[4] = 1;
      a.dwell[p] = best;
      a.dwell_ring[p] = best;
      a.trans[p] = (uint8_t)k;
      sh.s.move[c] = k | (gate ? 4 : 0);
      {
        unsigned long long b0, b1, b2, b3 = 0ull;
        if constexpr (MODE == kModeControl) {
          b0 = __ballot(alive && k == 3);
          b1 = __ballot(alive && k == 2);
          b2 = __ballot(alive && gate);
          b3 = __ballot(alive && k == 1);
        } else {
          b0 = __ballot(alive && k == 0);
          b1 = __ballot(alive && k == 1);
          b2 = __ballot(alive && k == 2);
        }
        if (c == 0) {
          if (b0) atomicAdd(&tally[0], (unsigned)__popcll(b0));
          if (b1) atomicAdd(&tally[1], (unsigned)__popcll(b1));
          if (b2) atomicAdd(&tally[2], (unsigned)__popcll(b2));
          if (b3) atomicAdd(&tally[3], (unsigned)__popcll(b3));
        }
      }
      const bool took_L = MODE == kModeControl ? (k & 1) : (k == 0);
      a.EX_out[p] = took_L ? EXL : EX0;
      a.EV_out[p] = took_L ? EVL : EV0;
      a.Hflf_out[p] = __builtin_nan("");
    }
    __syncthreads();
    pot64_finish<NB, REPLAY, MODE, false>(a, sh, p, alive, roff, w, c, h, v, g);
    __syncthreads();
    POT_ISTAMP(4);
  }
  __syncthreads();
  if (threadIdx.x == 0 && tally[4]) {
    a.ctl->failed = 1;
    a.ctl->failed_iter = a.iter;
  }
  if (threadIdx.x < 4 && tally[threadIdx.x]) atomicAdd(&a.stats[threadIdx.x], (unsigned long long)tally[threadIdx.x]);
```

mjhmc_amd/csrc/dense_pot64_kernels.hpp:

```cpp
#pragma once
#ifndef __HIPCC_RTC__
#include <hip/hip_runtime.h>
#endif
#include <stdint.h>

#include "dense_pot.hpp"
#include "dense_pot_tile.hpp"

namespace mjhmc {

template <int NB>
struct DVecN;
template <>
struct DVecN<1> {
  using type = double;
};
template <>
struct DVecN<2> {
  using type = __attribute__((ext_vector_type(2))) double;
};
template <>
struct DVecN<4> {
  using type = __attribute__((ext_vector_type(4))) double;
};
// ... 38 lines not shown

template <int NB>
struct Work {
  static constexpr int PB = NB == 1 ? 8 : 16;
  static constexpr int PQ = NB * 8 / PB;
  static constexpr unsigned kArea = 16u * PQ * 64u * PB;
  __amdgpu_buffer_rsrc_t rs;
  unsigned voff;
  static constexpr unsigned xb = 0;
  static constexpr unsigned vb = 4 * kArea;
};
template <int NB>
__device__ __forceinline__ Work<NB> work_of(double* scratch, unsigned wg, int w, int lane) {
  Work<NB> k;
  char* base = (char*)scratch + (size_t)wg * (8 * Work<NB>::kArea);
  k.rs = __builtin_amdgcn_make_buffer_rsrc((void*)base, 0, 8 * Work<NB>::kArea, 0x00020000);
  k.voff = (unsigned)w * Work<NB>::kArea + (unsigned)lane * Work<NB>::PB;
  return k;
}
using uvec4 = __attribute__((ext_vector_type(4))) unsigned;
using uvec2 = __attribute__((ext_vector_type(2))) unsigned;
using f64x2 = __attribute__((ext_vector_type(2))) double;
template <int NB>
__device__ __forceinline__ typename DVecN<NB>::type wk_load(const Work<NB>& k, unsigned area, int q) {
  if constexpr (NB == 1) {
    return __builtin_bit_cast(double, __builtin_amdgcn_raw_buffer_load_b64(k.rs, k.voff, area + (unsigned)q * 512u, 0));
  } else if constexpr (NB == 2) {
    return __builtin_bit_cast(f64x2, __builtin_amdgcn_raw_buffer_load_b128(k.rs, k.voff, area + (unsigned)q * 1024u, 0));
  } else {
    const f64x2 lo = __builtin_bit_cast(f64x2, __builtin_amdgcn_raw_buffer_load_b128(k.rs, k.voff, area + (unsigned)q * 2048u, 0));
    const f64x2 hi = __builtin_bit_cast(f64x2, __builtin_amdgcn_raw_buffer_load_b128(k.rs, k.voff, area + (unsigned)q * 2048u + 1024u, 0));
    typename DVecN<4>::type v;
    v[0] = lo[0];
    v[1] = lo[1];
    v[2] = hi[0];
    v[3] = hi[1];
    return v;
  }
}
template <int NB>
__device__ __forceinline__ void wk_store(const Work<NB>& k, unsigned area, int q, const typename DVecN<NB>::type& v) {
  if constexpr (NB == 1) {
    __builtin_amdgcn_raw_buffer_store_b64(__builtin_bit_cast(uvec2, v), k.rs, k.voff, area + (unsigned)q * 512u, 0);
  } else if constexpr (NB == 2) {
    __builtin_amdgcn_raw_buffer_store_b128(__builtin_bit_cast(uvec4, v), k.rs, k.voff, area + (unsigned)q * 1024u, 0);
  } else {
    f64x2 lo, hi;
    lo[0] = v[0];
    lo[1] = v[1];
    hi[0] = v[2];
    hi[1] = v[3];
    __builtin_amdgcn_raw_buffer_store_b128(__builtin_bit_cast(uvec4, lo), k.rs, k.voff, area + (unsigned)q * 2048u, 0);
    __builtin_amdgcn_raw_buffer_store_b128(__builtin_bit_cast(uvec4, hi), k.rs, k.voff, area + (unsigned)q * 2048u + 1024u, 0);
  }
}

template <int NB>
struct PieceOf {
  using type = uvec4;
};
template <>
struct PieceOf<1> {
  using type = unsigned long long;
};
template <int NB>
struct Stage {
  using P = typename PieceOf<NB>::type;
  static constexpr int PB = sizeof(P);
  static constexpr int RB = 1024 * NB;
  static constexpr int RP = RB / PB;
  static constexpr int K = 32 * RP / 256;
  static constexpr int KB = K < 16 ? K : 16;
};
__device__ __forceinline__ unsigned stage_addr(int row, int piece, int pb, int rb) {
  return (unsigned)(row * rb + ((piece ^ (row & 15)) * pb));
}
template <int NB>
__device__ __forceinline__ void stage_rows_in(const double* rows, int64_t p, char* img) {
  using S = Stage<NB>;
  using P = typename S::P;
  const int t = threadIdx.x;
#pragma unroll 1
  for (int i0 = 0; i0 < S::K; i0 += S::KB) {
    P buf[S::KB];
#pragma unroll
    for (int i = 0; i < S::KB; ++i) {
      const int k = (i0 + i) * 256 + t, row = k / S::RP, piece = k % S::RP;
      const int64_t pr = __shfl((long long)p, row);
      buf[i] = *reinterpret_cast<const P*>(reinterpret_cast<const char*>(rows) + (size_t)pr * S::RB + (size_t)piece * S::PB);
    }
#pragma unroll
    for (int i = 0; i < S::KB; ++i) {
      const int k = (i0 + i) * 256 + t, row = k / S::RP, piece = k % S::RP;
      *reinterpret_cast<P*>(img + stage_addr(row, piece, S::PB, S::RB)) = buf[i];
    }
  }
}
template <int NB>
__device__ __forceinline__ void stage_rows_out(double* rows, int64_t p, const char* img) {
  using S = Stage<NB>;
  using P = typename S::P;
  const int t = threadIdx.x;
#pragma unroll 1
  for (int i0 = 0; i0 < S::K; i0 += S::KB) {
#pragma unroll
    for (int i = 0; i < S::KB; ++i) {
      const int k = (i0 + i) * 256 + t, row = k / S::RP, piece = k % S::RP;
      const int64_t pr = __shfl((long long)p, row);
      *reinterpret_cast<P*>(reinterpret_cast<char*>(rows) + (size_t)pr * S::RB + (size_t)piece * S::PB) =
          *reinterpret_cast<const P*>(img + stage_addr(row, piece, S::PB, S::RB));
    }
  }
}
template <int NB>
__device__ __forceinline__ typename DVecN<NB>::type stage_get(const char* img, int w, int c, int h, int q) {
  using S = Stage<NB>;
  const int first = (8 * NB * (32 * w + acc_row(q, h))) / S::PB;
  if constexpr (NB == 4) {
    const f64x2 lo = *reinterpret_cast<const f64x2*>(img + stage_addr(c, first, S::PB, S::RB));
    const f64x2 hi = *reinterpret_cast<const f64x2*>(img + stage_addr(c, first + 1, S::PB, S::RB));
    typename DVecN<4>::type v;
    v[0] = lo[0];
    v[1] = lo[1];
    v[2] = hi[0];
    v[3] = hi[1];
    return v;
  } else {
    return *reinterpret_cast<const typename DVecN<NB>::type*>(img + stage_addr(c, first, S::PB, S::RB));
  }
}
template <int NB>
__device__ __forceinline__ void stage_put(char* img, int w, int c, int h, int q, const typename DVecN<NB>::type& v) {
  using S = Stage<NB>;
  const int first = (8 * NB * (32 * w + acc_row(q, h))) / S::PB;
  if constexpr (NB == 4) {
    f64x2 lo, hi;
    lo[0] = v[0];
    lo[1] = v[1];
    hi[0] = v[2];
    hi[1] = v[3];
    *reinterpret_cast<f64x2*>(img + stage_addr(c, first, S::PB, S::RB)) = lo;
    *reinterpret_cast<f64x2*>(img + stage_addr(c, first + 1, S::PB, S::RB)) = hi;
  } else {
    *reinterpret_cast<typename DVecN<NB>::type*>(img + stage_addr(c, first, S::PB, S::RB)) = v;
  }
}
template <int NB>
__device__ __forceinline__ char* stage_image(Shared<NB>& s) {
  static_assert(sizeof(s.pub) == 32 * Stage<NB>::RB, "the staging image is the two B-operand images");
  return reinterpret_cast<char*>(&s.pub[0][0]);
}

template <int NB>
struct VTile {
  double b[NB][16];
};

template <int NB, int NKICK>
__device__ __forceinline__ void kick_drift_pass(const Work<NB>& wk, const Tile<NB>& g, VTile<NB>& v, double c, double eps,
                                                PubWave<NB>* pub0, int w, int lane) {
  using DV = typename DVecN<NB>::type;
  DV xa[4], xb[4];
  auto load4 = [&](int q4, DV(&x)[4]) {
#pragma unroll
    for (int qq = 0; qq < 4; ++qq) x[qq] = wk_load<NB>(wk, wk.xb, 4 * q4 + qq);
  };
  auto kick4 = [&](int q4) {
#pragma unroll
    for (int qq = 0; qq < 4; ++qq) {
      const int q = 4 * q4 + qq;
#pragma unroll
      for (int r = 0; r < NB; ++r) {
        const double t = c * (double)g.b[r][q];
        double vv = v.b[r][q];
        vv = vv + t;
        if constexpr (NKICK == 2) vv = vv + t;
        v.b[r][q] = vv;
      }
    }
  };
  auto drift4 = [&](int q4, DV(&x)[4]) {
    f32x4 px[NB];
#pragma unroll
    for (int qq = 0; qq < 4; ++qq) {
      const int q = 4 * q4 + qq;
#pragma unroll
      for (int r = 0; r < NB; ++r) {
        const double xx = dget<NB>(x[qq], r) + eps * v.b[r][q];
        dset<NB>(x[qq], r, xx);
        px[r][qq] = (float)xx;
      }
      wk_store<NB>(wk, wk.xb, q, x[qq]);
    }
    if constexpr (NB == 4) {
      unsigned off = ((wk.voff >> 1) & 0xFFFFC000u) | (wk.voff & 0x3FFu);
      asm volatile("" : "+v"(off));
      char* img = reinterpret_cast<char*>(pub0) + off;
#pragma unroll
      for (int r = 0; r < NB; ++r) *reinterpret_cast<f32x4*>(img + (size_t)(r * 4 + q4) * 1024) = px[r];
    } else {
#pragma unroll
      for (int r = 0; r < NB; ++r) pub0[w].v[r][q4][lane] = px[r];
    }
  };
  load4(0, xa);
  load4(1, xb);
  __builtin_amdgcn_sched_barrier(0);
  kick4(0);
  drift4(0, xa);
  __builtin_amdgcn_sched_barrier(0);
  load4(2, xa);
  __builtin_amdgcn_sched_barrier(0);
  kick4(1);
  drift4(1, xb);
  __builtin_amdgcn_sched_barrier(0);
  load4(3, xb);
  __builtin_amdgcn_sched_barrier(0);
  kick4(2);
  drift4(2, xa);
  __builtin_amdgcn_sched_barrier(0);
  kick4(3);
  drift4(3, xb);
}

template <int NB>
__device__ __forceinline__ double closing_kick(const Tile<NB>& g, VTile<NB>& v, double c) {
  double s = 0.0;
#pragma unroll
  for (int q = 0; q < 16; ++q)
#pragma unroll
    for (int r = 0; r < NB; ++r) {
      const double vv = v.b[r][q] + c * (double)g.b[r][q];
      v.b[r][q] = vv;
      s = s + vv * vv;
    }
  return s;
}

template <int NB, class SH>
__device__ __forceinline__ double column_sum(SH& sh, int w, int c, int h, double part) {
  const double both = swap32_sum(part);
  if (h == 0) sh.red64[w][c] = both;
  __syncthreads();
  const double tot = sh.red64[0][c] + sh.red64[1][c] + sh.red64[2][c] + sh.red64[3][c];
  __syncthreads();
  return tot;
}

template <int NB>
__device__ __forceinline__ void staged_start(Shared<NB>& s, const Work<NB>& wk, const double* xin, const double* vin,
                                             const double* gin, int64_t p, int w, int c, int h, Tile<NB>& g, VTile<NB>& v,
                                             bool neg) {
  char* img = stage_image<NB>(s);
  stage_rows_in<NB>(xin, p, img);
  __syncthreads();
#pragma unroll
  for (int q = 0; q < 16; ++q) wk_store<NB>(wk, wk.xb, q, stage_get<NB>(img, w, c, h, q));
  __syncthreads();
  stage_rows_in<NB>(gin, p, img);
  __syncthreads();
#pragma unroll
  for (int q = 0; q < 16; ++q) {
    const typename DVecN<NB>::type gg = stage_get<NB>(img, w, c, h, q);
#pragma unroll
    for (int r = 0; r < NB; ++r) g.b[r][q] = (float)dget<NB>(gg, r);
  }
  __syncthreads();
  stage_rows_in<NB>(vin, p, img);
  __syncthreads();
#pragma unroll
  for (int q = 0; q < 16; ++q) {
    const typename DVecN<NB>::type vv = stage_get<NB>(img, w, c, h, q);
#pragma unroll
    for (int r = 0; r < NB; ++r) v.b[r][q] = neg ? -dget<NB>(vv, r) : dget<NB>(vv, r);
  }
  __syncthreads();
}

template <int NB>
__device__ __forceinline__ void staged_end_x(Shared<NB>& s, const Work<NB>& wk, double* xout, int64_t p, int w, int c, int h) {
  char* img = stage_image<NB>(s);
#pragma unroll
  for (int q = 0; q < 16; ++q) stage_put<NB>(img, w, c, h, q, wk_load<NB>(wk, wk.xb, q));
  __syncthreads();
  stage_rows_out<NB>(xout, p, img);
  __syncthreads();
}
template <int NB>
__device__ __forceinline__ void staged_end_vg(Shared<NB>& s, double* vout, double* gout, int64_t p, int w, int c, int h,
                                              const VTile<NB>& v, const Tile<NB>& g) {
  using DV = typename DVecN<NB>::type;
  char* img = stage_image<NB>(s);
#pragma unroll
  for (int q = 0; q < 16; ++q) {
    DV vv;
#pragma unroll
    for (int r = 0; r < NB; ++r) dset<NB>(vv, r, v.b[r][q]);
    stage_put<NB>(img, w, c, h, q, vv);
  }
  __syncthreads();
  stage_rows_out<NB>(vout, p, img);
  __syncthreads();
#pragma unroll
  for (int q = 0; q < 16; ++q) {
    DV gg;
#pragma unroll
    for (int r = 0; r < NB; ++r) dset<NB>(gg, r, (double)g.b[r][q]);
    stage_put<NB>(img, w, c, h, q, gg);
  }
  __syncthreads();
  stage_rows_out<NB>(gout, p, img);
  __syncthreads();
}

template <int NB, class XP>
__device__ __forceinline__ double pot64_trajectory(const PotModel& mdl, const XP& xp, AReg<NB>& ar, Shared64<NB>& sh, int w, int c, int h,
                                                   int lane, const Work<NB>& wk, Tile<NB>& g, VTile<NB>& v, int L, double eps,
                                                   double chalf, float* ex) {
  PubWave<NB>* pub0 = sh.s.pub[0];
  kick_drift_pass<NB, 1>(wk, g, v, chalf, eps, pub0, w, lane);
  for (int s = 0; s < L; ++s) {
    [[maybe_unused]] const int stamp_slot = s;
    POT_STAMP(0);
    if constexpr (NB == 4) {
#pragma unroll
      for (int k = 0; k < kPark / 2; ++k) {
        f64x2 two;
        two[0] = v.b[NB - 1][15 - 2 * k];
        two[1] = v.b[NB - 1][14 - 2 * k];
        sh.park[k][threadIdx.x] = __builtin_bit_cast(f32x4, two);
      }
    }
    pot_gradient_published<NB>(mdl, xp, ar, sh.s, w, c, h, lane, g, s == L - 1, ex, s);
    if constexpr (NB == 4) {
#pragma unroll
      for (int k = 0; k < kPark / 2; ++k) {
        const f64x2 two = __builtin_bit_cast(f64x2, sh.park[k][threadIdx.x]);
        v.b[NB - 1][15 - 2 * k] = two[0];
        v.b[NB - 1][14 - 2 * k] = two[1];
      }
#pragma unroll
      for (int r = 0; r < NB; ++r)
#pragma unroll
        for (int q = 0; q < 16; ++q) use_here(v.b[r][q]);
    }
    POT_STAMP(6);
    if (s < L - 1) kick_drift_pass<NB, 2>(wk, g, v, chalf, eps, pub0, w, lane);
    POT_STAMP(7);
  }
  const double part = closing_kick<NB>(g, v, chalf);
  return column_sum<NB>(sh, w, c, h, part) / 2.0;
}


template <int NB>
struct Finish64Shared {
  struct {
    int move[kP];
  } s;
  double red64[4][kP];
  double zn[128 * NB];
};

template <int NB, bool REPLAY, int MODE, bool FIX, class SH>
__device__ __forceinline__ void pot64_finish(const Pot64JumpArgs& a, SH& sh, int64_t p, bool alive, size_t roff, int w, int c,
                                             int h, const VTile<NB>& v, const Tile<NB>& g) {
  using DV = typename DVecN<NB>::type;
  const double* xin = a.X_in + roff;
  const double* vin = a.V_in + roff;
  const double* gin = a.G_in + roff;
  double* xo = a.X_out + roff;
  double* vo = a.V_out + roff;
  double* go = a.G_out + roff;
  const int mv = sh.s.move[c];
  const int k = mv & 3;
  bool take, flip, refresh;
  if constexpr (MODE == kModeControl) {
    const bool accept = k & 1, fl = k & 2;
    take = accept;
    flip = accept != fl;
    refresh = (mv & 4) != 0;
  } else {
    take = k == 0;
    flip = (MODE == kModeCT && k == 0) || k == 1;
    refresh = k == 2;
  }
  const bool tile_refreshes = __ballot(refresh) != 0ull;
  if (!FIX || !take) {
#pragma unroll
    for (int q = 0; q < 16; ++q) {
      DV gg;
      if (take) {
        if constexpr (!FIX) {
          DV vv;
#pragma unroll
          for (int r = 0; r < NB; ++r) {
            dset<NB>(vv, r, flip ? -v.b[r][q] : v.b[r][q]);
            dset<NB>(gg, r, (double)g.b[r][q]);
          }
          dv_store<NB>(vo, q, vv);
        }
      } else {
        gg = dv_load<NB>(gin, q);
        dv_store<NB>(xo, q, dv_load<NB>(xin, q));
      }
      dv_store<NB>(go, q, gg);
    }
  }
  double s2 = 0.0;
  if (!take || (REPLAY && refresh)) {
    const double* vsrc = take ? (const double*)vo : vin;
    const bool fl2 = flip && !take;
    const double* nrow = REPLAY ? lane_row<NB>(a.noise, alive ? p : 0, w, h) : nullptr;
#pragma unroll 1
    for (int q = 0; q < 16; ++q) {
      DV vv = dv_load<NB>(vsrc, q);
      if (fl2) vv = -vv;
      if constexpr (REPLAY) {
        if (refresh) {
          const DV z = dv_load<NB>(nrow, q);
#pragma unroll
          for (int r = 0; r < NB; ++r) {
            const double t = dget<NB>(vv, r) * a.r_keep + dget<NB>(z, r) * a.r_mix;
            dset<NB>(vv, r, t);
            s2 = s2 + t * t;
          }
        }
      }
      dv_store<NB>(vo, q, vv);
    }
  }
  if constexpr (!REPLAY) {
    unsigned cols = (unsigned)(__ballot(refresh) & 0xFFFFFFFFull);
    while (cols) {
      const int c0 = __ffs((int)cols) - 1;
      cols &= cols - 1;
      const int64_t p0 = __shfl((long long)p, c0);
      column_normals<NB, double>(a.key, (uint32_t)(a.first_pid + (p0 < a.N ? p0 : 0)), a.D, sh.zn);
      __syncthreads();
      if (c == c0) {
        const double* zrow = sh.zn + 32 * NB * w + 4 * NB * h;
#pragma unroll 1
        for (int q = 0; q < 16; ++q) {
          DV vv = dv_load<NB>(vo, q);
          const DV z = *reinterpret_cast<const DV*>(zrow + q_off<NB>(q));
#pragma unroll
          for (int r = 0; r < NB; ++r) {
            const double t = dget<NB>(vv, r) * a.r_keep + dget<NB>(z, r) * a.r_mix;
            dset<NB>(vv, r, t);
            s2 = s2 + t * t;
          }
          dv_store<NB>(vo, q, vv);
        }
      }
      __syncthreads();
    }
  }
  if (tile_refreshes) {
    const double evr = column_sum<NB>(sh, w, c, h, s2) / 2.0;
    if (refresh && w == 0 && h == 0) a.EV_out[p] = evr;
  }
}

template <bool REPLAY, int MODE>
__device__ __forceinline__ int pot64_decide(const Pot64JumpArgs& a, double H0, double HL, double Hflf, int64_t pp, uint32_t pid,
                                            double& best, bool& bad, bool& gate) {
  JumpArgs<double> ja;
  ja.p_r = a.p_r;
  ja.p_flip = a.p_flip;
  ja.rexp = a.rexp;
  ja.runif = a.runif;
  ja.N = a.N;
  LaneMap m;
  m.j = 0;
  m.G = 1;
  m.D = 1;
  m.CH = 1;
  m.lane0 = 0;
  m.wpp = 0;
  int k = 0;
  if constexpr (MODE == kModeMJHMC) {
    decide<double, REPLAY>(ja, a.key, m, H0, HL, Hflf, pp, pid, k, best, bad);
  } else if constexpr (MODE == kModeCT) {
    decide_ct<double, REPLAY>(ja, a.key, m, H0, HL, pp, pid, k, best, bad);
  } else {
    double uacc, uflip, ugate;
    if constexpr (REPLAY) {
      uacc = a.runif[pp];
      uflip = a.runif[a.N + pp];
      ugate = a.runif[2 * a.N];
    } else {
      const u32x4 q = philox4x32_10(pid, a.key.tick_lo, a.key.tick_hi, kSlotExpR, a.key.k0, a.key.k1);
      const u32x4 f = philox4x32_10(pid, a.key.tick_lo, a.key.tick_hi, kSlotFlip, a.key.k0, a.key.k1);
      const u32x4 gq = philox4x32_10(0xFFFFFFFFu, a.key.tick_lo, a.key.tick_hi, kSlotFlip, a.key.k0, a.key.k1);
      uacc = u53(q.w2, q.w3);
      uflip = u53(f.w0, f.w1);
      ugate = u53(gq.w2, gq.w3);
    }
    const double dH = H0 - HL;
    const bool accept = !(dH < 0.0) || (uacc < exp(dH));
    const bool flip = uflip < a.p_flip;
    gate = ugate < a.p_r;
    k = (accept ? 1 : 0) | (flip ? 2 : 0);
  }
  return k;
}


}
```

mjhmc_amd/csrc/handles.hpp:

```cpp
#pragma once
#include <hip/hip_runtime.h>

#include <string>
#include <vector>

#include "../../include/mjhmc_hip.h"
#include "dense_pot.hpp"
#include "dense_sic.hpp"
#include "elementwise.hpp"
#include "linear_energy.hpp"
#include "user_expr.hpp"

using namespace mjhmc;

int mjhmc_fail(int code, const std::string& msg);

#define HIPCHK(expr)                                                                                         \
  do {                                                                                                       \
    hipError_t e_ = (expr);                                                                                  \
    if (e_ != hipSuccess)                                                                                    \
      return mjhmc_fail(MJHMC_ERR_HIP, std::string(#expr) + ": " + hipGetErrorString(e_) + " (" + __FILE__ + \
                                           ":" + std::to_string(__LINE__) + ")");                            \
  } while (0)

#define TRY(expr)             \
  do {                        \
    int r_ = (expr);          \
    if (r_ != 0) return r_;   \
  } while (0)

struct mjhmc_ctx {
  int device;
  hipDeviceProp_t prop;
};

struct mjhmc_energy {
  mjhmc_ctx* ctx;
  EnergyParams ep;
  std::vector<double> params;
  void* dev64 = nullptr;
  void* dev32 = nullptr;
  float* pot[4] = {nullptr, nullptr, nullptr, nullptr};
  int pot_dim = kPotDim;
  int pot_rows = 0;
  PotModel pot_model() const { return PotModel{pot[0], pot[1], pot[2], pot[3], pot_dim, pot_rows ? pot_rows : ep.ndims}; }
  bool pot_big() const { return is_pot() && pot_dim > kPotDim; }
  PotBigModel pot_big_model() const { return PotBigModel{pot[0], pot[1], pot[2], pot[3], pot_dim, ep.ndims}; }
  bool is_pot() const { return ep.kind == MJHMC_E_PRODUCT_OF_T || ep.kind == MJHMC_E_LINEAR_EXPR; }
  LinearEnergy* lin = nullptr;
  const PotGenerated* pot_gen() const { return lin ? &lin->gen : nullptr; }
  void* sic[3] = {nullptr, nullptr, nullptr};
  float sic_lambda = 0.f;
  int sic_cauchy = 1;
  int sic_P = 1;
  int sic_copies = 1;
  int sic_nc = 1024;
  SicModel sic_model() const {
    return SicModel{sic[0], sic[1], (const float*)sic[2], sic_lambda, sic_cauchy, sic_P, 1.0f / (float)sic_P, sic_copies,
                    sic_nc};
  }
  bool is_sic() const { return ep.kind == MJHMC_E_SPARSE_CODE; }
  bool is_dense() const { return is_pot() || is_sic(); }
  UserEnergy* user = nullptr;
  bool is_user() const { return ep.kind == MJHMC_E_USER_EXPR; }
  bool is_host() const { return ep.kind == MJHMC_E_HOST; }
};

struct Shape {
  int E, logG, pitch, CH, esize;
  bool wide = false;
  bool round32 = false;
};


constexpr int kMaxDenseParts = 4;

struct mjhmc_estimator;
struct mjhmc_chainstats;
struct mjhmc_histogram;
struct mjhmc_pairhist;
struct mjhmc_functionals;
struct mjhmc_timegrid;
struct DlSession;
struct HostTraj;

struct mjhmc_sampler {
  mjhmc_ctx* ctx;
  mjhmc_energy* en;
  int64_t N, Npad, first_pid;
  int D, dtype, mode;
  Shape sh;
  hipStream_t stream = nullptr;
  char* h_pin = nullptr;
  size_t h_pin_cap = 0;
  std::vector<hipStream_t> part_streams;
  std::vector<hipEvent_t> part_events;
  hipEvent_t ev_join = nullptr;
  void* ick[7] = {nullptr, nullptr, nullptr, nullptr, nullptr, nullptr, nullptr};
  hipEvent_t ev_fork = nullptr;
  void* Xbuf[2] = {nullptr, nullptr};
  void* Vbuf[2] = {nullptr, nullptr};
  void* Xcur = nullptr;
  void* Gbuf[2] = {nullptr, nullptr};
  float* Hwork = nullptr;
  int* cold_list = nullptr;
  double* pot64_scratch = nullptr;
  void* Hspec[2] = {nullptr, nullptr};
  void* Hspec_dump = nullptr;
  int* flf_list = nullptr;
  bool list_valid = false;
  int list_par = 0;
  int list_count = 0;
  int* flf_counts = nullptr;
  void* Hpre = nullptr;
  int vcur = 0, scur = 0;
  void* EX[2] = {nullptr, nullptr};
  void* EV[2] = {nullptr, nullptr};
  void* Hflf[2] = {nullptr, nullptr};
  double* dwell = nullptr;
  double* dwell_scratch = nullptr;
  void* ck[7] = {nullptr, nullptr, nullptr, nullptr, nullptr, nullptr, nullptr};
  uint64_t ck_tick = 0;
  bool ck_valid = false;
  void* undo_X = nullptr;
  bool undo_valid = false;
  bool undo_multipass = false;
  uint8_t* trans = nullptr;
  char* call_block = nullptr;
  Control* ctl = nullptr;
  long long* stats = nullptr;
  int stats_cap = 0;
  void* ring = nullptr;
  double* dwell_ring = nullptr;
  int ring_slots = 0;
  uint64_t ring_gen = 0;
  std::vector<mjhmc_estimator*> estimators;
  std::vector<mjhmc_chainstats*> chainstats;
  std::vector<mjhmc_histogram*> histograms;
  std::vector<mjhmc_pairhist*> pairhists;
  std::vector<mjhmc_functionals*> functionals;
  std::vector<mjhmc_timegrid*> timegrids;
  double* stage = nullptr;
  size_t stage_elems = 0;
  void* noise = nullptr;
  double* rexp = nullptr;
  double* runif = nullptr;
  void* scratch = nullptr;
  bool download_f32 = false;
  double eps = 1e-4, p_r = 0, beta = 1, p_flip = 0.5;
  int L = 5;
  uint64_t seed = 0, tick = 1;
  hipEvent_t ev_total[2] = {nullptr, nullptr};
  std::vector<hipEvent_t> ev_k;
  double last_total_ms = 0, last_jump_ms = 0;
  int last_jump_launches = 0;
  bool timing_pending = false;
  bool timing_on = true;
  void* pipe_pin[2] = {nullptr, nullptr};
  hipEvent_t pipe_ev[2] = {nullptr, nullptr};
  DlSession* dl = nullptr;
  hipStream_t dl_stream = nullptr;
  double* dl_stage = nullptr;
  size_t dl_stage_elems = 0;
  void* dl_pin[2] = {nullptr, nullptr};
  hipEvent_t dl_ev[2] = {nullptr, nullptr};
  HostTraj* ht = nullptr;
  bool host_energy_set = false;
};

inline size_t row_bytes(const mjhmc_sampler* s) { return (size_t)s->sh.pitch * s->sh.esize; }
inline size_t ssize(const mjhmc_sampler* s) { return s->dtype == MJHMC_F64 ? 8 : 4; }
inline size_t mat_bytes(const mjhmc_sampler* s) { return (size_t)s->Npad * row_bytes(s); }


void estimator_free_all(mjhmc_sampler* s);

void chainstats_free_all(mjhmc_sampler* s);

void histogram_free_all(mjhmc_sampler* s);

void pairhist_free_all(mjhmc_sampler* s);

void functionals_free_all(mjhmc_sampler* s);

void timegrid_free_all(mjhmc_sampler* s);

void host_traj_free(mjhmc_sampler* s);
int host_run_eval(mjhmc_sampler* s, const void* V, void* Vgen, void* EVout);
int wide_run_eval(mjhmc_sampler* s, const void* X, void* Gout, void* Eout, const void* V, void* Vgen, void* EVout);
int multipass_iterate(mjhmc_sampler* s, int n_iter, const double* replay_normal, const double* replay_exp,
                      const double* replay_unif, int ring_slot0, mjhmc_iter_stats* per_iter, int* n_done);
int multipass_rollback(mjhmc_sampler* s);
int round_rows32(mjhmc_sampler* s, void* rows);
int wide_leapfrog(mjhmc_sampler* w, const double* X, const double* V, double* Xo, double* Vo, double* G, double* EX,
                  double* EV, double eps, int n_steps);

int pick_shape(int D, int dtype, Shape* out);
int ensure_stage(mjhmc_sampler* s, size_t elems);
int download_cols(mjhmc_sampler* s, const void* src, const int64_t* dev_idx, int64_t ncols, double* host,
                  size_t host_elems, int64_t rs, int64_t cs, int64_t off, bool copy_out);
int copy_to_host(mjhmc_sampler* s, const void* dev_src, void* host_dst, size_t bytes);
```

mjhmc_amd/csrc/host_energy.hip:

```cpp
#include <hip/hip_runtime.h>

#include <cmath>
#include <cstring>
#include <vector>

#include "handles.hpp"

struct HostTraj {
  double* X = nullptr;
  double* V = nullptr;
  double* G = nullptr;
  double* E = nullptr;
  double* EVw = nullptr;
  double* noise = nullptr;
  int* cold = nullptr;
  int* coldpos = nullptr;
  int* kmove = nullptr;
  double* dtmp = nullptr;
  double* hnew = nullptr;
  float* pot32[4] = {nullptr, nullptr, nullptr, nullptr};
  int n_cold = 0;
  int64_t n_cols = 0;
  int phase = 0;
  int steps = 0;
// ... 454 lines not shown
  a.key = RngKey{0u, 0u, 0u, 0u};
  pot_launch_eval(a, s->en->pot_model(), s->stream, s->en->pot_gen());
}

int pot_eval_rows_f64(mjhmc_sampler* s, const double* X, double* G, double* E, int64_t nrows) {
  const int pitch = s->sh.pitch;
  const int64_t rows_pad = (nrows + 63) / 64 * 64, ne = rows_pad * pitch;
  float* tmp[4] = {nullptr, nullptr, nullptr, nullptr};
  float** buf = tmp;
  const bool big = s->en->pot_big();
  const bool own = !(s->ht && rows_pad <= 2 * s->Npad);
  if (!own) {
    buf = s->ht->pot32;
    if (!buf[0]) {
      const size_t cap = (size_t)2 * s->Npad;
      HIPCHK(hipMalloc((void**)&buf[0], cap * pitch * sizeof(float)));
      HIPCHK(hipMalloc((void**)&buf[1], cap * pitch * sizeof(float)));
      HIPCHK(hipMalloc((void**)&buf[2], cap * sizeof(float)));
      if (big) HIPCHK(hipMalloc((void**)&buf[3], cap * pitch * sizeof(float)));
    }
  } else {
    HIPCHK(hipMalloc((void**)&buf[0], (size_t)ne * sizeof(float)));
    HIPCHK(hipMalloc((void**)&buf[1], (size_t)ne * sizeof(float)));
    HIPCHK(hipMalloc((void**)&buf[2], (size_t)rows_pad * sizeof(float)));
    if (big) HIPCHK(hipMalloc((void**)&buf[3], (size_t)ne * sizeof(float)));
  }
  auto body = [&]() -> int {
    HIPCHK(hipMemsetAsync(buf[0], 0, (size_t)ne * sizeof(float), s->stream));
    hipLaunchKernelGGL(hk_narrow, grid1(nrows * pitch), dim3(256), 0, s->stream, X, buf[0], nrows * pitch);
    pot_force32(s, buf, G != nullptr, E != nullptr, rows_pad, nrows);
    if (G) hipLaunchKernelGGL(hk_widen, grid1(nrows * pitch), dim3(256), 0, s->stream, (const float*)buf[1], G, nrows * pitch);
    if (E) hipLaunchKernelGGL(hk_widen, grid1(nrows), dim3(256), 0, s->stream, (const float*)buf[2], E, nrows);
    HIPCHK(hipGetLastError());
    if (own) HIPCHK(hipStreamSynchronize(s->stream));
    return 0;
  };
  const int rc = body();
  if (own)
    for (float* b : tmp)
      if (b) (void)hipFree(b);
  return rc;
}

int wide_eval_rows(mjhmc_sampler* s, const double* X, double* G, double* E, int64_t nrows) {
  if (s->en->is_pot()) return pot_eval_rows_f64(s, X, G, E, nrows);
  WideEnergy w;
  TRY(wide_energy_of(s->en, &w));
  hipLaunchKernelGGL(hk_energy_grad, dim3((unsigned)nrows), dim3(64), 0, s->stream, X, G, E, nrows, s->D, s->sh.pitch, w);
  HIPCHK(hipGetLastError());
  return 0;
}

int need_traj(mjhmc_sampler* s) {
  if (s->ht) return 0;
  HostTraj* t = new HostTraj();
  s->ht = t;
  const size_t rows = (size_t)2 * s->Npad, mb = rows * s->sh.pitch * sizeof(double);
  HIPCHK(hipMalloc((void**)&t->X, mb));
  HIPCHK(hipMalloc((void**)&t->V, mb));
  HIPCHK(hipMalloc((void**)&t->G, mb));
  HIPCHK(hipMemsetAsync(t->X, 0, mb, s->stream));
  HIPCHK(hipMemsetAsync(t->V, 0, mb, s->stream));
  HIPCHK(hipMemsetAsync(t->G, 0, mb, s->stream));
  HIPCHK(hipMalloc((void**)&t->E, rows * sizeof(double)));
  HIPCHK(hipMalloc((void**)&t->EVw, rows * sizeof(double)));
  HIPCHK(hipMalloc((void**)&t->cold, s->Npad * sizeof(int)));
  HIPCHK(hipMalloc((void**)&t->coldpos, s->Npad * sizeof(int)));
  HIPCHK(hipMalloc((void**)&t->kmove, s->Npad * sizeof(int)));
  HIPCHK(hipMalloc((void**)&t->dtmp, s->Npad * sizeof(double)));
  HIPCHK(hipMalloc((void**)&t->hnew, (size_t)3 * s->Npad * sizeof(double)));
  return 0;
}

int check_host(mjhmc_sampler* s) {
  if (!s) return mjhmc_fail(MJHMC_ERR_INVALID, "sampler is NULL");
  if (!s->en->is_host()) return mjhmc_fail(MJHMC_ERR_INVALID, "the sampler's energy is not MJHMC_E_HOST");
  return 0;
}

}

void host_traj_free(mjhmc_sampler* s) {
  HostTraj* t = s->ht;
  if (!t) return;
  void* bufs[] = {t->X, t->V, t->G, t->E, t->EVw, t->noise, t->cold, t->coldpos, t->kmove, t->dtmp, t->hnew,
                  t->pot32[0], t->pot32[1], t->pot32[2], t->pot32[3]};
  for (void* b : bufs)
    if (b) (void)hipFree(b);
  delete t;
  s->ht = nullptr;
}

int host_run_eval(mjhmc_sampler* s, const void* V, void* Vgen, void* EVout) {
  if (Vgen) {
    const RngKey key{(uint32_t)(s->seed & 0xFFFFFFFFu), (uint32_t)(s->seed >> 32), 0u, 0u};
    const int64_t n = s->N * ((s->D + 1) / 2);
    hipLaunchKernelGGL(hk_gen_v, grid1(n), dim3(256), 0, s->stream, (double*)Vgen, key, s->first_pid, s->N, s->D, s->sh.pitch);
    HIPCHK(hipGetLastError());
    V = Vgen;
  }
  if (V && EVout) {
    hipLaunchKernelGGL(hk_kinetic, dim3((unsigned)s->N), dim3(64), 0, s->stream, (const double*)V, (double*)EVout, s->N, s->D,
                       s->sh.pitch);
    HIPCHK(hipGetLastError());
  }
  return 0;
}

extern "C" {

int mjhmc_host_set_energy(mjhmc_sampler* s, const double* E, const double* dEdX) {
  TRY(check_host(s));
  if (!E || !dEdX) return mjhmc_fail(MJHMC_ERR_INVALID, "NULL argument");
  HIPCHK(hipSetDevice(s->ctx->device));
  HIPCHK(hipMemcpyAsync(s->EX[s->scur], E, (size_t)s->N * sizeof(double), hipMemcpyHostToDevice, s->stream));
  TRY(upload_rows(s, dEdX, s->N, (double*)s->Gbuf[s->vcur]));
  HIPCHK(hipStreamSynchronize(s->stream));
  s->host_energy_set = true;
  return 0;
}

int mjhmc_traj_begin(mjhmc_sampler* s, int64_t* n_cols) {
  TRY(check_host(s));
  if (!n_cols) return mjhmc_fail(MJHMC_ERR_INVALID, "n_cols is NULL");
  if (!s->host_energy_set)
    return mjhmc_fail(MJHMC_ERR_INVALID, "E and dE/dX of the current state are unknown: call mjhmc_host_set_energy first");
  HIPCHK(hipSetDevice(s->ctx->device));
  return traj_begin_impl(s, n_cols);
}

}

int traj_begin_impl(mjhmc_sampler* s, int64_t* n_cols) {
  TRY(need_traj(s));
  s->undo_valid = false;
  HostTraj* t = s->ht;
  const int pitch = s->sh.pitch;
  t->n_cold = 0;
  if (s->mode == MJHMC_MODE_MJHMC) {
    std::vector<double> h((size_t)s->N);
    HIPCHK(hipMemcpyAsync(h.data(), s->Hflf[s->scur], (size_t)s->N * sizeof(double), hipMemcpyDeviceToHost, s->stream));
    HIPCHK(hipStreamSynchronize(s->stream));
    std::vector<int> cold, pos((size_t)s->N, -1);
    for (int64_t p = 0; p < s->N; ++p)
      if (!(h[(size_t)p] == h[(size_t)p])) {
        pos[(size_t)p] = (int)cold.size();
        cold.push_back((int)p);
      }
    t->n_cold = (int)cold.size();
    if (t->n_cold) HIPCHK(hipMemcpyAsync(t->cold, cold.data(), cold.size() * sizeof(int), hipMemcpyHostToDevice, s->stream));
    HIPCHK(hipMemcpyAsync(t->coldpos, pos.data(), pos.size() * sizeof(int), hipMemcpyHostToDevice, s->stream));
    HIPCHK(hipStreamSynchronize(s->stream));
  }
  const double* X = (const double*)s->Xcur;
  const double* V = (const double*)s->Vbuf[s->vcur];
  const double* G = (const double*)s->Gbuf[s->vcur];
  const int64_t n1 = s->N * pitch;
  hipLaunchKernelGGL(hk_copy_rows, grid1(n1), dim3(256), 0, s->stream, t->X, X, (const int*)nullptr, s->N, pitch, 1.0);
  hipLaunchKernelGGL(hk_copy_rows, grid1(n1), dim3(256), 0, s->stream, t->V, V, (const int*)nullptr, s->N, pitch, 1.0);
  hipLaunchKernelGGL(hk_copy_rows, grid1(n1), dim3(256), 0, s->stream, t->G, G, (const int*)nullptr, s->N, pitch, 1.0);
  if (t->n_cold) {
    const int64_t n2 = (int64_t)t->n_cold * pitch;
    const size_t off = (size_t)s->N * pitch;
    hipLaunchKernelGGL(hk_copy_rows, grid1(n2), dim3(256), 0, s->stream, t->X + off, X, (const int*)t->cold, (int64_t)t->n_cold, pitch, 1.0);
    hipLaunchKernelGGL(hk_copy_rows, grid1(n2), dim3(256), 0, s->stream, t->V + off, V, (const int*)t->cold, (int64_t)t->n_cold, pitch, -1.0);
    hipLaunchKernelGGL(hk_copy_rows, grid1(n2), dim3(256), 0, s->stream, t->G + off, G, (const int*)t->cold, (int64_t)t->n_cold, pitch, 1.0);
  }
  HIPCHK(hipGetLastError());
  t->n_cols = s->N + t->n_cold;
  t->phase = 1;
  t->steps = 0;
  if (n_cols) *n_cols = t->n_cols;
  return 0;
}

extern "C" {

int mjhmc_traj_step(mjhmc_sampler* s, const double* grad, int last, double* X_out) {
  TRY(check_host(s));
  HostTraj* t = s->ht;
  if (!t || t->phase != 1) return mjhmc_fail(MJHMC_ERR_INVALID, "no trajectory in progress (mjhmc_traj_begin)");
  if (!last && !X_out) return mjhmc_fail(MJHMC_ERR_INVALID, "X_out is NULL");
  if (t->steps > 0 && !grad) return mjhmc_fail(MJHMC_ERR_INVALID, "the gradient at the positions handed out last is missing");
  HIPCHK(hipSetDevice(s->ctx->device));
  const int64_t n = t->n_cols, ne = n * s->sh.pitch;
  const double c = -s->eps / 2.;
  if (grad) {
    if (t->steps == 0) return mjhmc_fail(MJHMC_ERR_INVALID, "the first step uses the stored dE/dX: pass NULL");
    TRY(upload_rows(s, grad, n, t->G));
    hipLaunchKernelGGL(hk_axpy, grid1(ne), dim3(256), 0, s->stream, t->V, (const double*)t->G, c, ne);
  }
  if (!last) {
    hipLaunchKernelGGL(hk_axpy, grid1(ne), dim3(256), 0, s->stream, t->V, (const double*)t->G, c, ne);
    hipLaunchKernelGGL(hk_axpy, grid1(ne), dim3(256), 0, s->stream, t->X, (const double*)t->V, s->eps, ne);
    HIPCHK(hipGetLastError());
    t->steps += 1;
    TRY(ensure_stage(s, (size_t)s->D * n));
    return download_cols(s, t->X, nullptr, n, X_out, (size_t)s->D * n, n, 1, 0, true);
  }
  HIPCHK(hipGetLastError());
  t->phase = 2;
  return 0;
}

int mjhmc_traj_finish(mjhmc_sampler* s, const double* E, const double* replay_normal, const double* replay_exp,
                      const double* replay_unif, int ring_slot, mjhmc_iter_stats* st) {
  TRY(check_host(s));
  HostTraj* t = s->ht;
  if (!t || t->phase != 2) return mjhmc_fail(MJHMC_ERR_INVALID, "the trajectory is not complete (mjhmc_traj_step with last != 0)");
  if (!E) return mjhmc_fail(MJHMC_ERR_INVALID, "E is NULL");
  if (ring_slot >= s->ring_slots) return mjhmc_fail(MJHMC_ERR_INVALID, "ring slot out of range");
  HIPCHK(hipSetDevice(s->ctx->device));
  HIPCHK(hipMemcpyAsync(t->E, E, (size_t)t->n_cols * sizeof(double), hipMemcpyHostToDevice, s->stream));
  return traj_finish_impl(s, replay_normal, replay_exp, replay_unif, ring_slot, st);
}

}

int traj_finish_impl(mjhmc_sampler* s, const double* replay_normal, const double* replay_exp, const double* replay_unif,
                     int ring_slot, mjhmc_iter_stats* st) {
  HostTraj* t = s->ht;
  const int64_t n = t->n_cols;
  const int pitch = s->sh.pitch;
  const bool replay = s->mode == MJHMC_MODE_CONTROL ? (replay_unif != nullptr) : (replay_exp != nullptr);
  if (replay && !replay_normal) return mjhmc_fail(MJHMC_ERR_INVALID, "replay needs the normals as well");
  hipLaunchKernelGGL(hk_kinetic, dim3((unsigned)n), dim3(64), 0, s->stream, (const double*)t->V, t->EVw, n, s->D, pitch);
  if (replay) {
    if (!t->noise) HIPCHK(hipMalloc((void**)&t->noise, (size_t)s->Npad * pitch * sizeof(double)));
    TRY(upload_rows(s, replay_normal, s->N, t->noise));
    if (replay_exp) {
      if (!s->rexp) HIPCHK(hipMalloc((void**)&s->rexp, 3 * s->N * sizeof(double)));
      HIPCHK(hipMemcpyAsync(s->rexp, replay_exp, 3 * s->N * sizeof(double), hipMemcpyHostToDevice, s->stream));
    }
    if (replay_unif) {
      if (!s->runif) HIPCHK(hipMalloc((void**)&s->runif, (2 * s->N + 1) * sizeof(double)));
      HIPCHK(hipMemcpyAsync(s->runif, replay_unif, (2 * s->N + 1) * sizeof(double), hipMemcpyHostToDevice, s->stream));
    }
  }
  HIPCHK(hipMemsetAsync(s->ctl, 0, sizeof(Control), s->stream));
  HIPCHK(hipMemsetAsync(s->stats, 0, 4 * sizeof(long long), s->stream));
  const uint64_t tick = s->tick;
  const RngKey key{(uint32_t)(s->seed & 0xFFFFFFFFu), (uint32_t)(s->seed >> 32), (uint32_t)(tick & 0xFFFFFFFFu),
                   (uint32_t)(tick >> 32)};
  DecideArgs d;
  d.EX = (const double*)s->EX[s->scur];
  d.EV = (const double*)s->EV[s->scur];
  d.Hflf = (const double*)s->Hflf[s->scur];
  d.E = t->E;
  d.EVw = t->EVw;
  d.coldpos = t->coldpos;
  d.kmove = t->kmove;
  d.dtmp = t->dtmp;
  d.hnew = t->hnew;
  d.rexp = replay ? s->rexp : nullptr;
  d.runif = replay ? s->runif : nullptr;
  d.ctl = s->ctl;
  d.N = s->N;
  d.Npad = s->Npad;
  d.first_pid = s->first_pid;
  d.p_r = s->p_r;
  d.p_flip = s->p_flip;
  d.mode = s->mode;
  d.key = key;
  if (replay) hipLaunchKernelGGL(hk_decide<true>, grid1(s->N), dim3(256), 0, s->stream, d);
  else hipLaunchKernelGGL(hk_decide<false>, grid1(s->N), dim3(256), 0, s->stream, d);
  HIPCHK(hipGetLastError());
  Control hc;
  HIPCHK(hipMemcpyAsync(&hc, s->ctl, sizeof(Control), hipMemcpyDeviceToHost, s->stream));
  HIPCHK(hipStreamSynchronize(s->stream));
  s->tick += 1;
  t->phase = 0;
  long long hs[4] = {0, 0, 0, 0};
  if (!hc.failed) {
    CommitArgs c;
    c.X = (double*)s->Xcur;
    c.V = (double*)s->Vbuf[s->vcur];
    c.G = (double*)s->Gbuf[s->vcur];
    c.EXs = (double*)s->EX[s->scur];
    c.EVs = (double*)s->EV[s->scur];
    c.Hflf = (double*)s->Hflf[s->scur];
    c.TX = t->X;
    c.TV = t->V;
    c.TG = t->G;
    c.kmove = t->kmove;
    c.dtmp = t->dtmp;
    c.hnew = t->hnew;
    c.noise = replay ? t->noise : nullptr;
    c.dwell = s->dwell;
    c.dwell_ring = ring_slot >= 0 ? s->dwell_ring + (size_t)ring_slot * s->Npad : nullptr;
    c.trans = s->trans;
    c.ring_slot = ring_slot >= 0 ? (double*)((char*)s->ring + (size_t)ring_slot * mat_bytes(s)) : nullptr;
    c.stats = (unsigned long long*)s->stats;
    c.N = s->N;
    c.Npad = s->Npad;
    c.first_pid = s->first_pid;
    c.D = s->D;
    c.pitch = pitch;
    c.mode = s->mode;
    c.round32 = s->sh.round32 ? 1 : 0;
    c.r_keep = std::sqrt(1.0 - s->beta);
    c.r_mix = std::sqrt(s->beta);
    c.key = key;
    if (replay) hipLaunchKernelGGL(hk_commit<true>, dim3((unsigned)s->N), dim3(64), 0, s->stream, c);
    else hipLaunchKernelGGL(hk_commit<false>, dim3((unsigned)s->N), dim3(64), 0, s->stream, c);
    HIPCHK(hipGetLastError());
    if (s->sh.round32 && !s->en->is_host()) {
      TRY(wide_eval_rows(s, (const double*)s->Xcur, (double*)s->Gbuf[s->vcur], (double*)s->EX[s->scur], s->N));
      hipLaunchKernelGGL(hk_kinetic, dim3((unsigned)s->N), dim3(64), 0, s->stream, (const double*)s->Vbuf[s->vcur],
                         (double*)s->EV[s->scur], s->N, s->D, pitch);
      HIPCHK(hipGetLastError());
    }
    HIPCHK(hipMemcpyAsync(hs, s->stats, sizeof(hs), hipMemcpyDeviceToHost, s->stream));
    HIPCHK(hipStreamSynchronize(s->stream));
  }
  s->undo_valid = !hc.failed;
  s->undo_multipass = true;
  if (st) {
    std::memset(st, 0, sizeof(*st));
    if (s->mode == MJHMC_MODE_MJHMC) {
      st->l = hs[0];
      st->f = hs[1];
      st->r = hs[2];
      st->n_cold = t->n_cold;
    } else if (s->mode == MJHMC_MODE_CTHMC) {
      st->fl = hs[0];
      st->f = hs[1];
      st->r = hs[2];
    } else {
      st->l = hs[0];
      st->f = hs[1];
      st->r = hs[2];
      st->fl = hs[3];
    }
    st->E_evals = n;
    st->dEdX_evals = (int64_t)t->steps * n;
    st->nonfinite = hc.failed ? 1 : 0;
    st->L_used = t->steps;
    st->eps_used = s->eps;
    st->n_flf_run = st->n_cold;
  }
  return 0;
}

int multipass_rollback(mjhmc_sampler* s) {
  HostTraj* t = s->ht;
  if (!t) return mjhmc_fail(MJHMC_ERR_INVALID, "nothing to roll back");
  HIPCHK(hipSetDevice(s->ctx->device));
  hipLaunchKernelGGL(hk_undo, dim3((unsigned)s->N), dim3(64), 0, s->stream, (double*)s->Xcur, (double*)s->Vbuf[s->vcur],
                     (double*)s->Gbuf[s->vcur], (double*)s->EX[s->scur], (double*)s->EV[s->scur], (double*)s->Hflf[s->scur],
                     (const double*)t->X, (const double*)t->V, (const double*)t->G, (const double*)t->hnew, s->N, s->Npad, s->D,
                     s->sh.pitch);
  HIPCHK(hipGetLastError());
  HIPCHK(hipStreamSynchronize(s->stream));
  return 0;
}


int wide_run_eval(mjhmc_sampler* s, const void* X, void* Gout, void* Eout, const void* V, void* Vgen, void* EVout) {
  if (!s->en->is_host() && X && (Gout || Eout)) TRY(wide_eval_rows(s, (const double*)X, (double*)Gout, (double*)Eout, s->N));
  return host_run_eval(s, V, Vgen, EVout);
}

static int traj_advance(mjhmc_sampler* s, bool closing_kick, bool last) {
  HostTraj* t = s->ht;
  const int64_t ne = t->n_cols * s->sh.pitch;
  const double c = -s->eps / 2.;
  if (closing_kick) hipLaunchKernelGGL(hk_axpy, grid1(ne), dim3(256), 0, s->stream, t->V, (const double*)t->G, c, ne);
  if (!last) {
    hipLaunchKernelGGL(hk_axpy, grid1(ne), dim3(256), 0, s->stream, t->V, (const double*)t->G, c, ne);
    hipLaunchKernelGGL(hk_axpy, grid1(ne), dim3(256), 0, s->stream, t->X, (const double*)t->V, s->eps, ne);
    t->steps += 1;
  }
  HIPCHK(hipGetLastError());
  return 0;
}

static int pot_trajectory_f64(mjhmc_sampler* s) {
  HostTraj* t = s->ht;
  const int pitch = s->sh.pitch;
  const int64_t n = t->n_cols, rows_pad = (n + 63) / 64 * 64, ne = n * pitch;
  if (!t->pot32[0]) {
    const size_t cap = (size_t)2 * s->Npad;
    HIPCHK(hipMalloc((void**)&t->pot32[0], cap * pitch * sizeof(float)));
    HIPCHK(hipMalloc((void**)&t->pot32[1], cap * pitch * sizeof(float)));
    HIPCHK(hipMalloc((void**)&t->pot32[2], cap * sizeof(float)));
    if (s->en->pot_big()) HIPCHK(hipMalloc((void**)&t->pot32[3], cap * pitch * sizeof(float)));
  }
  HIPCHK(hipMemsetAsync(t->pot32[0], 0, (size_t)rows_pad * pitch * sizeof(float), s->stream));
  const double c = -s->eps / 2.;
  for (int l = 0; l < s->L; ++l) {
    if (l == 0)
      hipLaunchKernelGGL(hk_pot_kick_drift<false>, grid1(ne), dim3(256), 0, s->stream, t->X, t->V, (const void*)t->G, t->pot32[0], c,
                         s->eps, 0, ne);
    else
      hipLaunchKernelGGL(hk_pot_kick_drift<true>, grid1(ne), dim3(256), 0, s->stream, t->X, t->V, (const void*)t->pot32[1],
                         t->pot32[0], c, s->eps, 1, ne);
    pot_force32(s, t->pot32, true, l == s->L - 1, rows_pad, n);
    t->steps += 1;
  }
  hipLaunchKernelGGL(hk_pot_close, grid1(ne), dim3(256), 0, s->stream, t->V, (const float*)t->pot32[1], t->G, c, ne);
  hipLaunchKernelGGL(hk_widen, grid1(n), dim3(256), 0, s->stream, (const float*)t->pot32[2], t->E, n);
  HIPCHK(hipGetLastError());
  return 0;
}

int multipass_iterate(mjhmc_sampler* s, int n_iter, const double* replay_normal, const double* replay_exp,
                      const double* replay_unif, int ring_slot0, mjhmc_iter_stats* per_iter, int* n_done) {
  const size_t DN = (size_t)s->D * s->N;
  int done = 0;
  if (s->timing_on) HIPCHK(hipEventRecord(s->ev_total[0], s->stream));
  for (int i = 0; i < n_iter; ++i) {
    TRY(traj_begin_impl(s, nullptr));
    HostTraj* t = s->ht;
    if (s->en->is_pot() && s->L > 0) {
      TRY(pot_trajectory_f64(s));
    } else {
      for (int l = 0; l < s->L; ++l) {
        TRY(traj_advance(s, l > 0, false));
        TRY(wide_eval_rows(s, t->X, t->G, l == s->L - 1 ? t->E : nullptr, t->n_cols));
      }
      TRY(traj_advance(s, s->L > 0, true));
      if (s->L == 0) TRY(wide_eval_rows(s, t->X, nullptr, t->E, t->n_cols));
    }
    t->phase = 2;
    mjhmc_iter_stats st;
    TRY(traj_finish_impl(s, replay_normal ? replay_normal + (size_t)i * DN : nullptr,
                         replay_exp ? replay_exp + (size_t)i * 3 * s->N : nullptr,
                         replay_unif ? replay_unif + (size_t)i * (2 * s->N + 1) : nullptr,
                         ring_slot0 >= 0 ? ring_slot0 + i : -1, &st));
    if (per_iter) per_iter[i] = st;
    if (st.nonfinite) break;
    done += 1;
  }
  if (s->timing_on) HIPCHK(hipEventRecord(s->ev_total[1], s->stream));
  s->undo_valid = (n_iter == 1 && done == 1);
  s->last_jump_launches = std::min(done + 1, n_iter);
  s->timing_pending = s->timing_on;
  if (n_done) *n_done = done;
  return 0;
}

int wide_leapfrog(mjhmc_sampler* w, const double* X, const double* V, double* Xo, double* Vo, double* G, double* EX,
                  double* EV, double eps, int n_steps) {
  const int64_t ne = w->Npad * w->sh.pitch, nv = w->N * w->sh.pitch;
  double* g = G;
  if (!g) HIPCHK(hipMalloc((void**)&g, (size_t)ne * sizeof(double)));
  auto body = [&]() -> int {
    HIPCHK(hipMemcpyAsync(Xo, X, (size_t)ne * sizeof(double), hipMemcpyDeviceToDevice, w->stream));
    HIPCHK(hipMemcpyAsync(Vo, V, (size_t)ne * sizeof(double), hipMemcpyDeviceToDevice, w->stream));
    TRY(wide_eval_rows(w, Xo, g, EX, w->N));
    const double c = -eps / 2.;
    for (int l = 0; l < n_steps; ++l) {
      hipLaunchKernelGGL(hk_axpy, grid1(nv), dim3(256), 0, w->stream, Vo, (const double*)g, c, nv);
      hipLaunchKernelGGL(hk_axpy, grid1(nv), dim3(256), 0, w->stream, Xo, (const double*)Vo, eps, nv);
      TRY(wide_eval_rows(w, Xo, g, EX, w->N));
      hipLaunchKernelGGL(hk_axpy, grid1(nv), dim3(256), 0, w->stream, Vo, (const double*)g, c, nv);
    }
    if (w->sh.round32) {
      TRY(round_rows32(w, Xo));
      TRY(round_rows32(w, Vo));
      TRY(wide_eval_rows(w, Xo, g, EX, w->N));
    }
    if (EV) hipLaunchKernelGGL(hk_kinetic, dim3((unsigned)w->N), dim3(64), 0, w->stream, (const double*)Vo, EV, w->N, w->D, w->sh.pitch);
    HIPCHK(hipGetLastError());
    HIPCHK(hipStreamSynchronize(w->stream));
    return 0;
  };
  const int rc = body();
  if (!G && g) (void)hipFree(g);
  return rc;
}
```

Measured before the change: 62.24 billion.

## Store V and dE/dX in wave-tiled layout with f32 gradient

Switches the persistent V and gradient buffers of the f64 dense-potential path to a per-wave tiled layout that matches the kernel's register tiles, and stores the gradient as f32 at half the size. The fused kernel then loads and stores V/G directly per lane, dropping the shared-memory staging round trips and barriers in staged_start and staged_end. Host-facing paths (upload, download, multipass, rollback) untile and retile through new row-major scratch buffers. The extra conversion kernels on those paths add cost there, and keeping the gradient in f32 gives up precision that was formerly held in double.

```diff
diff --git a/mjhmc_amd/csrc/api.hip b/mjhmc_amd/csrc/api.hip
--- a/mjhmc_amd/csrc/api.hip
+++ b/mjhmc_amd/csrc/api.hip
@@ -356,6 +356,19 @@
   s->stage_elems = 0;
   HIPCHK(hipMalloc(&s->stage, elems * sizeof(double)));
   s->stage_elems = elems;
+  return 0;
+}
+
+int vg_untile(mjhmc_sampler* s) {
+  for (int i = 0; i < 2; ++i)
+    if (!s->vg_rows[i]) HIPCHK(hipMalloc((void**)&s->vg_rows[i], mat_bytes(s)));
+  pot64_vg_retile(s->sh.pitch, s->Npad, false, s->vg_rows[0], s->vg_rows[1], s->Vbuf[s->vcur], s->Gbuf[s->vcur], s->stream);
+  HIPCHK(hipGetLastError());
+  return 0;
+}
+int vg_retile(mjhmc_sampler* s) {
+  pot64_vg_retile(s->sh.pitch, s->Npad, true, s->vg_rows[0], s->vg_rows[1], s->Vbuf[s->vcur], s->Gbuf[s->vcur], s->stream);
+  HIPCHK(hipGetLastError());
   return 0;
 }
 
@@ -969,7 +982,7 @@
   histogram_free_all(s);
   pairhist_free_all(s);
   timegrid_free_all(s);
-  void* ptrs[] = {s->flf_list, s->call_block, s->Hpre, s->Hwork, s->cold_list, s->pot64_scratch, s->Hspec[0], s->Hspec[1], s->Hspec_dump, s->Gbuf[0], s->Gbuf[1], s->Xbuf[0], s->Xbuf[1], s->Vbuf[0],  s->Vbuf[1], s->EX[0],     s->EX[1],  s->EV[0],
+  void* ptrs[] = {s->vg_rows[0], s->vg_rows[1], s->flf_list, s->call_block, s->Hpre, s->Hwork, s->cold_list, s->pot64_scratch, s->Hspec[0], s->Hspec[1], s->Hspec_dump, s->Gbuf[0], s->Gbuf[1], s->Xbuf[0], s->Xbuf[1], s->Vbuf[0],  s->Vbuf[1], s->EX[0],     s->EX[1],  s->EV[0],
                   s->EV[1],   s->Hflf[0], s->Hflf[1],  s->dwell,  s->dwell_scratch,  s->trans,
                   s->ring,     s->dwell_ring, s->stage,  s->noise,  s->rexp,
                   s->runif,   s->scratch,  s->ck[0],    s->ck[1],    s->ck[2],   s->ck[3],  s->ck[4],
@@ -1042,8 +1055,8 @@
       HIPCHK(hipMemsetAsync(s->Xbuf[i], 0, mb, s->stream));
       HIPCHK(hipMemsetAsync(s->Vbuf[i], 0, mb, s->stream));
       if (e->is_pot() || ((e->is_host() || s->sh.wide) && i == 0)) {
-        HIPCHK(hipMalloc(&s->Gbuf[i], mb));
-        HIPCHK(hipMemsetAsync(s->Gbuf[i], 0, mb, s->stream));
+        HIPCHK(hipMalloc(&s->Gbuf[i], dedx_bytes(s)));
+        HIPCHK(hipMemsetAsync(s->Gbuf[i], 0, dedx_bytes(s), s->stream));
       }
       if (e->is_dense()) {
         if (!s->Hwork) {
@@ -1075,17 +1088,22 @@
     s->Xcur = s->Xbuf[0];
     TRY(upload_matrix(s, Xinit, s->Xcur));
     if (s->sh.round32) TRY(round_rows32(s, s->Xcur));
+    const bool tiled = vg_tiled(s);
+    if (tiled) TRY(vg_untile(s));
+    void* const Vrows = tiled ? (void*)s->vg_rows[0] : s->Vbuf[0];
+    void* const Grows = tiled ? (void*)s->vg_rows[1] : s->Gbuf[0];
     if (Vinit) {
-      TRY(upload_matrix(s, Vinit, s->Vbuf[0]));
-      if (s->sh.round32) TRY(round_rows32(s, s->Vbuf[0]));
-      TRY(run_eval(s, s->Xcur, s->Gbuf[0], s->EX[0], s->Vbuf[0], nullptr, s->EV[0]));
+      TRY(upload_matrix(s, Vinit, Vrows));
+      if (s->sh.round32) TRY(round_rows32(s, Vrows));
+      TRY(run_eval(s, s->Xcur, Grows, s->EX[0], Vrows, nullptr, s->EV[0]));
     } else {
-      TRY(run_eval(s, s->Xcur, s->Gbuf[0], s->EX[0], nullptr, s->Vbuf[0], s->EV[0]));
+      TRY(run_eval(s, s->Xcur, Grows, s->EX[0], nullptr, Vrows, s->EV[0]));
       if (s->sh.round32) {
-        TRY(round_rows32(s, s->Vbuf[0]));
-        TRY(run_eval(s, nullptr, nullptr, nullptr, s->Vbuf[0], nullptr, s->EV[0]));
+        TRY(round_rows32(s, Vrows));
+        TRY(run_eval(s, nullptr, nullptr, nullptr, Vrows, nullptr, s->EV[0]));
       }
     }
+    if (tiled) TRY(vg_retile(s));
     HIPCHK(hipStreamSynchronize(s->stream));
     return 0;
   };
@@ -1125,7 +1143,7 @@
   HIPCHK(hipSetDevice(s->ctx->device));
   const size_t mb = mat_bytes(s), vb = (size_t)s->Npad * ssize(s), db = (size_t)s->Npad * sizeof(double);
   const int nck = (s->en->is_pot() || s->en->is_host() || s->sh.wide) ? 7 : 6;
-  const size_t sizes[7] = {mb, mb, vb, vb, vb, db, mb};
+  const size_t sizes[7] = {mb, mb, vb, vb, vb, db, dedx_bytes(s)};
   const void* src[7] = {s->Xcur, s->Vbuf[s->vcur], s->EX[s->scur], s->EV[s->scur], s->Hflf[s->scur], s->dwell,
                         s->Gbuf[s->vcur]};
   for (int i = 0; i < nck; ++i) {
@@ -1143,7 +1161,7 @@
   HIPCHK(hipSetDevice(s->ctx->device));
   const size_t mb = mat_bytes(s), vb = (size_t)s->Npad * ssize(s), db = (size_t)s->Npad * sizeof(double);
   const int nck = (s->en->is_pot() || s->en->is_host() || s->sh.wide) ? 7 : 6;
-  const size_t sizes[7] = {mb, mb, vb, vb, vb, db, mb};
+  const size_t sizes[7] = {mb, mb, vb, vb, vb, db, dedx_bytes(s)};
   s->Xcur = s->Xbuf[0];
   void* dst[7] = {s->Xcur, s->Vbuf[s->vcur], s->EX[s->scur], s->EV[s->scur], s->Hflf[s->scur], s->dwell,
                   s->Gbuf[s->vcur]};
@@ -1258,8 +1276,9 @@
     h.next_count = counters + 3 * which + (a.iter + 1) % 3;
     h.zero_count = counters + 3 * which + (a.iter + 2) % 3;
     if constexpr (A::kPot) {
-      h.G_in = a.G_in + (size_t)start * pitch;
-      h.G_out = a.G_out + (size_t)start * pitch;
+      const size_t gpitch = A::kScratch ? pitch / 2 : pitch;
+      h.G_in = a.G_in + (size_t)start * gpitch;
+      h.G_out = a.G_out + (size_t)start * gpitch;
     }
     if constexpr (A::kScratch)
       h.scratch = a.scratch + (size_t)which * pot64_scratch_workgroups() * 2 * 32 * (size_t)pitch;
@@ -1289,7 +1308,7 @@
 static int split_state_copy(mjhmc_sampler* s, bool restore) {
   const size_t mb = mat_bytes(s), vb = (size_t)s->Npad * ssize(s), db = (size_t)s->Npad * sizeof(double);
   const int nck = s->en->is_pot() ? 7 : 6;
-  const size_t sizes[7] = {mb, mb, vb, vb, vb, db, mb};
+  const size_t sizes[7] = {mb, mb, vb, vb, vb, db, dedx_bytes(s)};
   void* live[7] = {s->Xcur, s->Vbuf[s->vcur], s->EX[s->scur], s->EV[s->scur], s->Hflf[s->scur], s->dwell, s->Gbuf[s->vcur]};
   for (int i = 0; i < nck; ++i) {
     if (!s->ick[i]) HIPCHK(hipMalloc(&s->ick[i], sizes[i]));
@@ -1931,7 +1950,10 @@
       if (nbytes != mat * sizeof(double)) return fail(MJHMC_ERR_INVALID, "expected (D,N) float64");
       TRY(ensure_stage(s, mat));
       const void* src = field == MJHMC_F_X ? s->Xcur : s->Vbuf[s->vcur];
-      if (field == MJHMC_F_DEDX && (s->en->is_pot() || s->en->is_host() || s->sh.wide)) {
+      if (field != MJHMC_F_X && vg_tiled(s)) {
+        TRY(vg_untile(s));
+        src = s->vg_rows[field == MJHMC_F_V ? 0 : 1];
+      } else if (field == MJHMC_F_DEDX && (s->en->is_pot() || s->en->is_host() || s->sh.wide)) {
         src = s->Gbuf[s->vcur];
       } else if (field == MJHMC_F_DEDX && s->en->is_sic()) {
         if (!s->scratch) HIPCHK(hipMalloc(&s->scratch, (size_t)s->Npad * s->D * sizeof(float)));
@@ -1986,13 +2008,18 @@
     case MJHMC_F_X:
     case MJHMC_F_V: {
       if (nbytes != mat * sizeof(double)) return fail(MJHMC_ERR_INVALID, "expected (D,N) float64");
-      void* dst = field == MJHMC_F_X ? s->Xcur : s->Vbuf[s->vcur];
+      const bool tiled = vg_tiled(s);
+      if (tiled) TRY(vg_untile(s));
+      void* const Vrows = tiled ? (void*)s->vg_rows[0] : s->Vbuf[s->vcur];
+      void* const Grows = tiled ? (void*)s->vg_rows[1] : s->Gbuf[s->vcur];
+      void* dst = field == MJHMC_F_X ? s->Xcur : Vrows;
       s->undo_valid = false;
       s->list_valid = false;
       if (field == MJHMC_F_X) s->host_energy_set = false;
       TRY(upload_matrix(s, (const double*)host_src, dst));
       if (s->sh.round32) TRY(round_rows32(s, dst));
-      TRY(run_eval(s, s->Xcur, s->Gbuf[s->vcur], s->EX[s->scur], s->Vbuf[s->vcur], nullptr, s->EV[s->scur]));
+      TRY(run_eval(s, s->Xcur, Grows, s->EX[s->scur], Vrows, nullptr, s->EV[s->scur]));
+      if (tiled) TRY(vg_retile(s));
       HIPCHK(hipMemsetAsync(s->Hflf[s->scur], 0xFF, s->Npad * ssize(s), s->stream));
       TRY(drop_spec(s));
       HIPCHK(hipStreamSynchronize(s->stream));
diff --git a/mjhmc_amd/csrc/dense_pot.hpp b/mjhmc_amd/csrc/dense_pot.hpp
--- a/mjhmc_amd/csrc/dense_pot.hpp
+++ b/mjhmc_amd/csrc/dense_pot.hpp
@@ -165,6 +165,7 @@
   void* params[] = {(void*)&a, (void*)&mdl, (void*)&lin};
   (void)hipModuleLaunchKernel(f, grid, 1, 1, 256, 1, 1, 0, st, params, nullptr);
 }
+void pot64_vg_retile(int dim, int64_t npad, bool to_tiles, double* vrows, double* grows, void* vtile, void* gtile, hipStream_t st);
 int pot64_scratch_workgroups();
 #endif
 
diff --git a/mjhmc_amd/csrc/dense_pot64.hip b/mjhmc_amd/csrc/dense_pot64.hip
--- a/mjhmc_amd/csrc/dense_pot64.hip
+++ b/mjhmc_amd/csrc/dense_pot64.hip
@@ -91,6 +91,39 @@
   if (threadIdx.x < 4 && tally[threadIdx.x]) atomicAdd(&a.stats[threadIdx.x], (unsigned long long)tally[threadIdx.x]);
 }
 
+__host__ __device__ inline int64_t tile_index(int nb, bool dedx, int64_t p, int d) {
+  const int w = d / (32 * nb), rem = d % (32 * nb), row = rem / nb, r = rem % nb;
+  const int h = (row >> 2) & 1, q = (row & 3) + 4 * (row >> 3);
+  const int64_t lane = (p & 31) + 32 * h;
+  const int64_t tile0 = (p >> 5) * (32 * 128 * (int64_t)nb);
+  if (dedx) return tile0 + (int64_t)w * (1024 * nb) + ((4 * r + (q >> 2)) * 64 + lane) * 4 + (q & 3);
+  const int ep = nb == 1 ? 1 : 2, pq = nb == 4 ? 2 : 1;
+  return tile0 + (int64_t)w * (1024 * nb) + ((q * pq + r / ep) * 64 + lane) * ep + r % ep;
+}
+
+__global__ void vg_rows_kernel(double* __restrict__ vrows, double* __restrict__ grows, double* __restrict__ vtile,
+                               float* __restrict__ gtile, int nb, int64_t n_elems, int to_tiles) {
+  const int64_t i = (int64_t)blockIdx.x * blockDim.x + threadIdx.x;
+  if (i >= n_elems) return;
+  const int dim = 128 * nb;
+  const int64_t p = i / dim;
+  const int d = (int)(i % dim);
+  const int64_t iv = tile_index(nb, false, p, d), ig = tile_index(nb, true, p, d);
+  if (to_tiles) {
+    vtile[iv] = vrows[i];
+    gtile[ig] = (float)grows[i];
+  } else {
+    vrows[i] = vtile[iv];
+    grows[i] = (double)gtile[ig];
+  }
+}
+
+void pot64_vg_retile(int dim, int64_t npad, bool to_tiles, double* vrows, double* grows, void* vtile, void* gtile, hipStream_t st) {
+  const int64_t n = npad * dim;
+  hipLaunchKernelGGL(vg_rows_kernel, dim3((unsigned)((n + 255) / 256)), dim3(256), 0, st, vrows, grows, (double*)vtile,
+                     (float*)gtile, dim / 128, n, to_tiles ? 1 : 0);
+}
+
 static int resident_cus64() {
   int dev = 0, cus = 0;
   (void)hipGetDevice(&dev);
@@ -135,6 +168,13 @@
   else launch64_nb<4>(a, mdl, st, gen);
 }
 
+}
+extern "C" long long mjhmc_pot64_tile_index(int nb, int dedx, long long p, int d) {
+  if ((nb != 1 && nb != 2 && nb != 4) || p < 0 || d < 0 || d >= 128 * nb) return -1;
+  return mjhmc::tile_index(nb, dedx != 0, p, d);
+}
+namespace mjhmc {
+
 #ifdef POT_STAMPS
 }
 extern "C" int mjhmc_pot64_stamps(unsigned long long* out) {
diff --git a/mjhmc_amd/csrc/dense_pot64_jump.inc b/mjhmc_amd/csrc/dense_pot64_jump.inc
--- a/mjhmc_amd/csrc/dense_pot64_jump.inc
+++ b/mjhmc_amd/csrc/dense_pot64_jump.inc
@@ -31,7 +31,7 @@
     {
       const int64_t p = column_of(item);
       POT_ISTAMP(0);
-      staged_start<NB>(sh.s, wk, a.X_in, a.V_in, a.G_in, p, w, c, h, g, v, inverse);
+      staged_start<NB>(sh.s, wk, a.X_in, a.V_in, reinterpret_cast<const float*>(a.G_in), p, w, c, h, g, v, inverse);
       POT_ISTAMP(1);
       EVL = pot64_trajectory<NB>(mdl, xp, ar, sh, w, c, h, lane, wk, g, v, a.L, a.eps, a.chalf, &exl);
       POT_ISTAMP(2);
@@ -57,7 +57,7 @@
         a.EX_out[p] = EXL;
         a.EV_out[p] = EVL;
       }
-      staged_end_vg<NB>(sh.s, a.V_out, a.G_out, p, w, c, h, v, g);
+      tile_store_vg<NB>(a.V_out, reinterpret_cast<float*>(a.G_out), p, w, h, v, g);
       POT_ISTAMP(4);
       continue;
     }
diff --git a/mjhmc_amd/csrc/dense_pot64_kernels.hpp b/mjhmc_amd/csrc/dense_pot64_kernels.hpp
--- a/mjhmc_amd/csrc/dense_pot64_kernels.hpp
+++ b/mjhmc_amd/csrc/dense_pot64_kernels.hpp
@@ -214,6 +214,79 @@
 }
 
 template <int NB>
+struct TileVG {
+  static constexpr int PB = Work<NB>::PB, PQ = Work<NB>::PQ;
+  static constexpr size_t kVWave = Work<NB>::kArea;
+  static constexpr size_t kVTile = 4 * kVWave;
+  static constexpr size_t kGWave = 4096 * NB;
+  static constexpr size_t kGTile = 4 * kGWave;
+};
+template <int NB, class C>
+__device__ __forceinline__ C* tv_lane(C* base, int64_t p, int w, int h) {
+  using T = TileVG<NB>;
+  return base + (size_t)(p >> 5) * T::kVTile + (size_t)w * T::kVWave + (size_t)(((int)p & 31) + 32 * h) * T::PB;
+}
+template <int NB, class C>
+__device__ __forceinline__ C* tg_lane(C* base, int64_t p, int w, int h) {
+  using T = TileVG<NB>;
+  return base + (size_t)(p >> 5) * T::kGTile + (size_t)w * T::kGWave + (size_t)(((int)p & 31) + 32 * h) * 16;
+}
+template <int NB, class C>
+__device__ __forceinline__ C* tv_lane_fwd(C* base, int64_t p, int w, int h) {
+  using T = TileVG<NB>;
+  const size_t tile = (size_t)__builtin_amdgcn_readfirstlane((int)(p >> 5));
+  return base + tile * T::kVTile + ((unsigned)w * (unsigned)T::kVWave + (unsigned)(((int)p & 31) + 32 * h) * (unsigned)T::PB);
+}
+template <int NB, class C>
+__device__ __forceinline__ C* tg_lane_fwd(C* base, int64_t p, int w, int h) {
+  using T = TileVG<NB>;
+  const size_t tile = (size_t)__builtin_amdgcn_readfirstlane((int)(p >> 5));
+  return base + tile * T::kGTile + ((unsigned)w * (unsigned)T::kGWave + (unsigned)(((int)p & 31) + 32 * h) * 16u);
+}
+template <int NB>
+__device__ __forceinline__ typename DVecN<NB>::type tv_load(const char* lane, int q) {
+  if constexpr (NB == 1) {
+    return *reinterpret_cast<const double*>(lane + q * 512);
+  } else if constexpr (NB == 2) {
+    return *reinterpret_cast<const f64x2*>(lane + q * 1024);
+  } else {
+    const f64x2 lo = *reinterpret_cast<const f64x2*>(lane + q * 2048);
+    const f64x2 hi = *reinterpret_cast<const f64x2*>(lane + q * 2048 + 1024);
+    typename DVecN<4>::type v;
+    v[0] = lo[0];
+    v[1] = lo[1];
+    v[2] = hi[0];
+    v[3] = hi[1];
+    return v;
+  }
+}
+template <int NB>
+__device__ __forceinline__ void tv_store(char* lane, int q, const typename DVecN<NB>::type& v) {
+  if constexpr (NB == 1) {
+    *reinterpret_cast<double*>(lane + q * 512) = v;
+  } else if constexpr (NB == 2) {
+    *reinterpret_cast<f64x2*>(lane + q * 1024) = v;
+  } else {
+    f64x2 lo, hi;
+    lo[0] = v[0];
+    lo[1] = v[1];
+    hi[0] = v[2];
+    hi[1] = v[3];
+    *reinterpret_cast<f64x2*>(lane + q * 2048) = lo;
+    *reinterpret_cast<f64x2*>(lane + q * 2048 + 1024) = hi;
+  }
+}
+__device__ __forceinline__ f32x4 tg_load(const char* lane, int k) { return *reinterpret_cast<const f32x4*>(lane + k * 1024); }
+__device__ __forceinline__ void tg_store(char* lane, int k, const f32x4& v) { *reinterpret_cast<f32x4*>(lane + k * 1024) = v; }
+template <int NB>
+__device__ __forceinline__ f32x4 tg_piece(const Tile<NB>& g, int k) {
+  f32x4 t;
+#pragma unroll
+  for (int j = 0; j < 4; ++j) t[j] = g.b[k >> 2][4 * (k & 3) + j];
+  return t;
+}
+
+template <int NB>
 struct VTile {
   double b[NB][16];
 };
@@ -311,32 +384,35 @@
 
 template <int NB>
 __device__ __forceinline__ void staged_start(Shared<NB>& s, const Work<NB>& wk, const double* xin, const double* vin,
-                                             const double* gin, int64_t p, int w, int c, int h, Tile<NB>& g, VTile<NB>& v,
+                                             const float* gin, int64_t p, int w, int c, int h, Tile<NB>& g, VTile<NB>& v,
                                              bool neg) {
   char* img = stage_image<NB>(s);
   stage_rows_in<NB>(xin, p, img);
+  __builtin_amdgcn_sched_barrier(0);
+  const char* vl = tv_lane<NB>(reinterpret_cast<const char*>(vin), p, w, h);
+  const char* gl = tg_lane<NB>(reinterpret_cast<const char*>(gin), p, w, h);
+#pragma unroll
+  for (int q = 0; q < 16; ++q) {
+    const typename DVecN<NB>::type vv = tv_load<NB>(vl, q);
+#pragma unroll
+    for (int r = 0; r < NB; ++r) v.b[r][q] = dget<NB>(vv, r);
+  }
   __syncthreads();
 #pragma unroll
   for (int q = 0; q < 16; ++q) wk_store<NB>(wk, wk.xb, q, stage_get<NB>(img, w, c, h, q));
   __syncthreads();
-  stage_rows_in<NB>(gin, p, img);
-  __syncthreads();
-#pragma unroll
-  for (int q = 0; q < 16; ++q) {
-    const typename DVecN<NB>::type gg = stage_get<NB>(img, w, c, h, q);
-#pragma unroll
-    for (int r = 0; r < NB; ++r) g.b[r][q] = (float)dget<NB>(gg, r);
-  }
-  __syncthreads();
-  stage_rows_in<NB>(vin, p, img);
-  __syncthreads();
-#pragma unroll
-  for (int q = 0; q < 16; ++q) {
-    const typename DVecN<NB>::type vv = stage_get<NB>(img, w, c, h, q);
-#pragma unroll
-    for (int r = 0; r < NB; ++r) v.b[r][q] = neg ? -dget<NB>(vv, r) : dget<NB>(vv, r);
-  }
-  __syncthreads();
+#pragma unroll
+  for (int k = 0; k < 4 * NB; ++k) {
+    const f32x4 t = tg_load(gl, k);
+#pragma unroll
+    for (int j = 0; j < 4; ++j) g.b[k >> 2][4 * (k & 3) + j] = t[j];
+  }
+  if (neg) {
+#pragma unroll
+    for (int q = 0; q < 16; ++q)
+#pragma unroll
+      for (int r = 0; r < NB; ++r) v.b[r][q] = -v.b[r][q];
+  }
 }
 
 template <int NB>
@@ -349,30 +425,20 @@
   __syncthreads();
 }
 template <int NB>
-__device__ __forceinline__ void staged_end_vg(Shared<NB>& s, double* vout, double* gout, int64_t p, int w, int c, int h,
-                                              const VTile<NB>& v, const Tile<NB>& g) {
-  using DV = typename DVecN<NB>::type;
-  char* img = stage_image<NB>(s);
+__device__ __forceinline__ void tile_store_vg(double* vout, float* gout, int64_t p, int w, int h, const VTile<NB>& v,
+                                              const Tile<NB>& g) {
+  char* vl = tv_lane_fwd<NB>(reinterpret_cast<char*>(vout), p, w, h);
 #pragma unroll
   for (int q = 0; q < 16; ++q) {
-    DV vv;
+    typename DVecN<NB>::type vv;
 #pragma unroll
     for (int r = 0; r < NB; ++r) dset<NB>(vv, r, v.b[r][q]);
-    stage_put<NB>(img, w, c, h, q, vv);
-  }
-  __syncthreads();
-  stage_rows_out<NB>(vout, p, img);
-  __syncthreads();
-#pragma unroll
-  for (int q = 0; q < 16; ++q) {
-    DV gg;
-#pragma unroll
-    for (int r = 0; r < NB; ++r) dset<NB>(gg, r, (double)g.b[r][q]);
-    stage_put<NB>(img, w, c, h, q, gg);
-  }
-  __syncthreads();
-  stage_rows_out<NB>(gout, p, img);
-  __syncthreads();
+    tv_store<NB>(vl, q, vv);
+  }
+  __builtin_amdgcn_sched_barrier(0);
+  char* gl = tg_lane_fwd<NB>(reinterpret_cast<char*>(gout), p, w, h);
+#pragma unroll
+  for (int k = 0; k < 4 * NB; ++k) tg_store(gl, k, tg_piece<NB>(g, k));
 }
 
 template <int NB, class XP>
@@ -429,11 +495,11 @@
                                              int h, const VTile<NB>& v, const Tile<NB>& g) {
   using DV = typename DVecN<NB>::type;
   const double* xin = a.X_in + roff;
-  const double* vin = a.V_in + roff;
-  const double* gin = a.G_in + roff;
   double* xo = a.X_out + roff;
-  double* vo = a.V_out + roff;
-  double* go = a.G_out + roff;
+  const char* vin = tv_lane_fwd<NB>(reinterpret_cast<const char*>(a.V_in), p, w, h);
+  const char* gin = tg_lane_fwd<NB>(reinterpret_cast<const char*>(a.G_in), p, w, h);
+  char* vo = tv_lane_fwd<NB>(reinterpret_cast<char*>(a.V_out), p, w, h);
+  char* go = tg_lane_fwd<NB>(reinterpret_cast<char*>(a.G_out), p, w, h);
   const int mv = sh.s.move[c];
   const int k = mv & 3;
   bool take, flip, refresh;
@@ -448,35 +514,32 @@
     refresh = k == 2;
   }
   const bool tile_refreshes = __ballot(refresh) != 0ull;
-  if (!FIX || !take) {
-#pragma unroll
-    for (int q = 0; q < 16; ++q) {
-      DV gg;
-      if (take) {
-        if constexpr (!FIX) {
-          DV vv;
-#pragma unroll
-          for (int r = 0; r < NB; ++r) {
-            dset<NB>(vv, r, flip ? -v.b[r][q] : v.b[r][q]);
-            dset<NB>(gg, r, (double)g.b[r][q]);
-          }
-          dv_store<NB>(vo, q, vv);
-        }
-      } else {
-        gg = dv_load<NB>(gin, q);
-        dv_store<NB>(xo, q, dv_load<NB>(xin, q));
+  if (take) {
+    if constexpr (!FIX) {
+#pragma unroll
+      for (int q = 0; q < 16; ++q) {
+        DV vv;
+#pragma unroll
+        for (int r = 0; r < NB; ++r) dset<NB>(vv, r, flip ? -v.b[r][q] : v.b[r][q]);
+        tv_store<NB>(vo, q, vv);
       }
-      dv_store<NB>(go, q, gg);
-    }
+#pragma unroll
+      for (int k = 0; k < 4 * NB; ++k) tg_store(go, k, tg_piece<NB>(g, k));
+    }
+  } else {
+#pragma unroll
+    for (int q = 0; q < 16; ++q) dv_store<NB>(xo, q, dv_load<NB>(xin, q));
+#pragma unroll
+    for (int k = 0; k < 4 * NB; ++k) tg_store(go, k, tg_load(gin, k));
   }
   double s2 = 0.0;
   if (!take || (REPLAY && refresh)) {
-    const double* vsrc = take ? (const double*)vo : vin;
+    const char* vsrc = take ? (const char*)vo : vin;
     const bool fl2 = flip && !take;
     const double* nrow = REPLAY ? lane_row<NB>(a.noise, alive ? p : 0, w, h) : nullptr;
 #pragma unroll 1
     for (int q = 0; q < 16; ++q) {
-      DV vv = dv_load<NB>(vsrc, q);
+      DV vv = tv_load<NB>(vsrc, q);
       if (fl2) vv = -vv;
       if constexpr (REPLAY) {
         if (refresh) {
@@ -489,7 +552,7 @@
           }
         }
       }
-      dv_store<NB>(vo, q, vv);
+      tv_store<NB>(vo, q, vv);
     }
   }
   if constexpr (!REPLAY) {
@@ -504,7 +567,7 @@
         const double* zrow = sh.zn + 32 * NB * w + 4 * NB * h;
 #pragma unroll 1
         for (int q = 0; q < 16; ++q) {
-          DV vv = dv_load<NB>(vo, q);
+          DV vv = tv_load<NB>(vo, q);
           const DV z = *reinterpret_cast<const DV*>(zrow + q_off<NB>(q));
 #pragma unroll
           for (int r = 0; r < NB; ++r) {
@@ -512,7 +575,7 @@
             dset<NB>(vv, r, t);
             s2 = s2 + t * t;
           }
-          dv_store<NB>(vo, q, vv);
+          tv_store<NB>(vo, q, vv);
         }
       }
       __syncthreads();
diff --git a/mjhmc_amd/csrc/handles.hpp b/mjhmc_amd/csrc/handles.hpp
--- a/mjhmc_amd/csrc/handles.hpp
+++ b/mjhmc_amd/csrc/handles.hpp
@@ -102,6 +102,7 @@
   void* Vbuf[2] = {nullptr, nullptr};
   void* Xcur = nullptr;
   void* Gbuf[2] = {nullptr, nullptr};
+  double* vg_rows[2] = {nullptr, nullptr};
   float* Hwork = nullptr;
   int* cold_list = nullptr;
   double* pot64_scratch = nullptr;
@@ -171,6 +172,8 @@
 inline size_t row_bytes(const mjhmc_sampler* s) { return (size_t)s->sh.pitch * s->sh.esize; }
 inline size_t ssize(const mjhmc_sampler* s) { return s->dtype == MJHMC_F64 ? 8 : 4; }
 inline size_t mat_bytes(const mjhmc_sampler* s) { return (size_t)s->Npad * row_bytes(s); }
+inline bool vg_tiled(const mjhmc_sampler* s) { return s->sh.wide && s->en->is_pot() && !s->en->pot_big() && !s->sh.round32; }
+inline size_t dedx_bytes(const mjhmc_sampler* s) { return vg_tiled(s) ? mat_bytes(s) / 2 : mat_bytes(s); }
 
 
 void estimator_free_all(mjhmc_sampler* s);
@@ -191,6 +194,8 @@
 int multipass_iterate(mjhmc_sampler* s, int n_iter, const double* replay_normal, const double* replay_exp,
                       const double* replay_unif, int ring_slot0, mjhmc_iter_stats* per_iter, int* n_done);
 int multipass_rollback(mjhmc_sampler* s);
+int vg_untile(mjhmc_sampler* s);
+int vg_retile(mjhmc_sampler* s);
 int round_rows32(mjhmc_sampler* s, void* rows);
 int wide_leapfrog(mjhmc_sampler* w, const double* X, const double* V, double* Xo, double* Vo, double* G, double* EX,
                   double* EV, double eps, int n_steps);
diff --git a/mjhmc_amd/csrc/host_energy.hip b/mjhmc_amd/csrc/host_energy.hip
--- a/mjhmc_amd/csrc/host_energy.hip
+++ b/mjhmc_amd/csrc/host_energy.hip
@@ -630,9 +630,11 @@
     HIPCHK(hipMemcpyAsync(t->coldpos, pos.data(), pos.size() * sizeof(int), hipMemcpyHostToDevice, s->stream));
     HIPCHK(hipStreamSynchronize(s->stream));
   }
+  const bool tiled = vg_tiled(s);
+  if (tiled) TRY(vg_untile(s));
   const double* X = (const double*)s->Xcur;
-  const double* V = (const double*)s->Vbuf[s->vcur];
-  const double* G = (const double*)s->Gbuf[s->vcur];
+  const double* V = tiled ? s->vg_rows[0] : (const double*)s->Vbuf[s->vcur];
+  const double* G = tiled ? s->vg_rows[1] : (const double*)s->Gbuf[s->vcur];
   const int64_t n1 = s->N * pitch;
   hipLaunchKernelGGL(hk_copy_rows, grid1(n1), dim3(256), 0, s->stream, t->X, X, (const int*)nullptr, s->N, pitch, 1.0);
   hipLaunchKernelGGL(hk_copy_rows, grid1(n1), dim3(256), 0, s->stream, t->V, V, (const int*)nullptr, s->N, pitch, 1.0);
@@ -752,8 +754,9 @@
   if (!hc.failed) {
     CommitArgs c;
     c.X = (double*)s->Xcur;
-    c.V = (double*)s->Vbuf[s->vcur];
-    c.G = (double*)s->Gbuf[s->vcur];
+    const bool tiled = vg_tiled(s);
+    c.V = tiled ? s->vg_rows[0] : (double*)s->Vbuf[s->vcur];
+    c.G = tiled ? s->vg_rows[1] : (double*)s->Gbuf[s->vcur];
     c.EXs = (double*)s->EX[s->scur];
     c.EVs = (double*)s->EV[s->scur];
     c.Hflf = (double*)s->Hflf[s->scur];
@@ -788,6 +791,7 @@
                          (double*)s->EV[s->scur], s->N, s->D, pitch);
       HIPCHK(hipGetLastError());
     }
+    if (tiled) TRY(vg_retile(s));
     HIPCHK(hipMemcpyAsync(hs, s->stats, sizeof(hs), hipMemcpyDeviceToHost, s->stream));
     HIPCHK(hipStreamSynchronize(s->stream));
   }
@@ -824,11 +828,14 @@
   HostTraj* t = s->ht;
   if (!t) return mjhmc_fail(MJHMC_ERR_INVALID, "nothing to roll back");
   HIPCHK(hipSetDevice(s->ctx->device));
-  hipLaunchKernelGGL(hk_undo, dim3((unsigned)s->N), dim3(64), 0, s->stream, (double*)s->Xcur, (double*)s->Vbuf[s->vcur],
-                     (double*)s->Gbuf[s->vcur], (double*)s->EX[s->scur], (double*)s->EV[s->scur], (double*)s->Hflf[s->scur],
+  const bool tiled = vg_tiled(s);
+  if (tiled) TRY(vg_untile(s));
+  hipLaunchKernelGGL(hk_undo, dim3((unsigned)s->N), dim3(64), 0, s->stream, (double*)s->Xcur,
+                     tiled ? s->vg_rows[0] : (double*)s->Vbuf[s->vcur], tiled ? s->vg_rows[1] : (double*)s->Gbuf[s->vcur], (double*)s->EX[s->scur], (double*)s->EV[s->scur], (double*)s->Hflf[s->scur],
                      (const double*)t->X, (const double*)t->V, (const double*)t->G, (const double*)t->hnew, s->N, s->Npad, s->D,
                      s->sh.pitch);
   HIPCHK(hipGetLastError());
+  if (tiled) TRY(vg_retile(s));
   HIPCHK(hipStreamSynchronize(s->stream));
   return 0;
 }
```

Result: no change. 62.46 billion (median of 6 runs) (+0.3%).
